# vocdoni/zk-franchise-proof-circuit

Measured on AMD Instinct MI355X. Metric: zkCensus proofs/sec (nLevels=160), higher is better.
Workload: dtype u256 (8 x u32 Montgomery, BN254 Fr/Fq)

## Files before the change

### zk-franchise-proof-circuit_amd/csrc/zkc_f29.h

```cpp
#pragma once
#include "zkc_field.h"

namespace zkc {

constexpr uint32_t F29_MASK = (1u << 29) - 1;
struct L9 { uint32_t l[9]; };

namespace f29_detail {
struct Big { uint64_t d[10]; };
constexpr Big big_norm(Big a) { uint64_t c = 0; for (int i = 0; i < 10; i++) { uint64_t v = a.d[i] + c; a.d[i] = v & F29_MASK; c = v >> 29; } return a; }
constexpr bool big_ge(const Big& a, const Big& b) { for (int i = 9; i >= 0; i--) { if (a.d[i] != b.d[i]) return a.d[i] > b.d[i]; } return true; }
constexpr Big big_sub(Big a, const Big& b) {
    int64_t br = 0;
    for (int i = 0; i < 10; i++) { int64_t v = (int64_t)a.d[i] - (int64_t)b.d[i] - br; br = v < 0; a.d[i] = (uint64_t)(v + (br ? (int64_t)1 << 29 : 0)); }
    return a;
}
constexpr Big big_shl1(Big a) { for (int i = 0; i < 10; i++) a.d[i] <<= 1; return big_norm(a); }
template <class P> constexpr Big big_p() { Big r{}; for (int k = 0; k < 9; k++) r.d[k] = P29<P>::limb(k); return r; }
template <class P> constexpr Big big_mod(Big a) {
    Big sh[40] = {}; sh[0] = big_p<P>(); int top = 0;
    for (int s = 1; s < 36; s++) { sh[s] = big_shl1(sh[s - 1]); top = s; }
    for (int s = top; s >= 0; s--) if (big_ge(a, sh[s])) a = big_sub(a, sh[s]);
    return a;
}
}

template <class P> constexpr L9 f29_p() { L9 r{}; for (int k = 0; k < 9; k++) r.l[k] = P29<P>::limb(k); return r; }
template <class P> constexpr L9 f29_dominator(uint32_t minlimb, uint32_t toplimb) {
    using namespace f29_detail;
    Big t{}; for (int i = 0; i < 8; i++) t.d[i] = minlimb; t.d[8] = toplimb;
    Big r = big_mod<P>(big_norm(t));
    bool zero = true; for (int i = 0; i < 10; i++) zero = zero && r.d[i] == 0;
    Big delta = zero ? r : big_sub(big_p<P>(), r);
    L9 o{}; for (int i = 0; i < 8; i++) o.l[i] = minlimb + (uint32_t)delta.d[i]; o.l[8] = toplimb + (uint32_t)delta.d[8];
    return o;
}
template <class P> constexpr L9 f29_pow2(int k) {
    using namespace f29_detail;
    Big t{}; t.d[k / 29] = 1ull << (k % 29);
    Big r = big_mod<P>(t);
    L9 o{}; for (int i = 0; i < 9; i++) o.l[i] = (uint32_t)r.d[i];
    return o;
}

template <class P> struct F29K {
    static constexpr L9 p = f29_p<P>();
    static constexpr L9 one = f29_pow2<P>(261);
    static constexpr L9 dom1 = f29_dominator<P>(1u << 29, 1u << 27);
    static constexpr L9 dom3 = f29_dominator<P>(3u << 29, 1u << 27);
    static constexpr uint32_t ninv = P::inv & F29_MASK;
    static constexpr uint32_t pinv = (0u - P::inv) & F29_MASK;
};

ZKC_HD void f29_from_fp_shl5(uint32_t r[9], const uint32_t a[8]) {
    r[0] = slice29<-5>(a); r[1] = slice29<24>(a); r[2] = slice29<53>(a); r[3] = slice29<82>(a); r[4] = slice29<111>(a);
    r[5] = slice29<140>(a); r[6] = slice29<169>(a); r[7] = slice29<198>(a); r[8] = slice29<227>(a);
}
ZKC_HD void f29_carry(uint32_t a[9]) {
#pragma unroll
    for (int k = 0; k < 8; k++) { a[k + 1] += a[k] >> 29; a[k] &= F29_MASK; }
}
ZKC_HD void f29_add(uint32_t r[9], const uint32_t a[9], const uint32_t b[9]) {
#pragma unroll
    for (int k = 0; k < 9; k++) r[k] = a[k] + b[k];
}
ZKC_HD void f29_sub(uint32_t r[9], const uint32_t a[9], const uint32_t b[9], const L9& D) {
#pragma unroll
    for (int k = 0; k < 9; k++) r[k] = a[k] + D.l[k] - b[k];
}

template <class P>
ZKC_HD void f29_mul(uint32_t r[9], const uint32_t a[9], const uint32_t b[9]) {
    constexpr L9 Pl = F29K<P>::p;
    uint64_t c[18];
#pragma unroll
    for (int k = 0; k < 18; k++) c[k] = 0;
#pragma unroll
    for (int i = 0; i < 9; i++)
#pragma unroll
        for (int j = 0; j < 9; j++) c[i + j] += (uint64_t)a[i] * b[j];
    uint64_t carry = 0;
#pragma unroll
    for (int i = 0; i < 9; i++) {
        c[i] += carry;
        const uint32_t m = ((uint32_t)c[i] * F29K<P>::ninv) & F29_MASK;
#pragma unroll
        for (int j = 0; j < 9; j++) c[i + j] += (uint64_t)m * Pl.l[j];
        carry = c[i] >> 29;
    }
#pragma unroll
    for (int k = 9; k < 17; k++) { c[k] += carry; r[k - 9] = (uint32_t)c[k] & F29_MASK; carry = c[k] >> 29; }
    r[8] = (uint32_t)(c[17] + carry);
}
template <class P>
ZKC_HD void f29_sqr(uint32_t r[9], const uint32_t a[9]) {
    constexpr L9 Pl = F29K<P>::p;
    uint64_t c[18];
    uint32_t a2[9];
#pragma unroll
    for (int k = 0; k < 9; k++) a2[k] = a[k] << 1;
#pragma unroll
    for (int k = 0; k < 18; k++) c[k] = 0;
#pragma unroll
    for (int i = 0; i < 9; i++) {
        c[2 * i] += (uint64_t)a[i] * a[i];
#pragma unroll
        for (int j = i + 1; j < 9; j++) c[i + j] += (uint64_t)a2[i] * a[j];
    }
    uint64_t carry = 0;
#pragma unroll
    for (int i = 0; i < 9; i++) {
        c[i] += carry;
        const uint32_t m = ((uint32_t)c[i] * F29K<P>::ninv) & F29_MASK;
#pragma unroll
        for (int j = 0; j < 9; j++) c[i + j] += (uint64_t)m * Pl.l[j];
        carry = c[i] >> 29;
    }
#pragma unroll
    for (int k = 9; k < 17; k++) { c[k] += carry; r[k - 9] = (uint32_t)c[k] & F29_MASK; carry = c[k] >> 29; }
    r[8] = (uint32_t)(c[17] + carry);
}

template <class P>
ZKC_HD void f29_reduce_cols(uint32_t r[9], uint64_t c[18]) {
    constexpr L9 Pl = F29K<P>::p;
    uint64_t carry = 0;
#pragma unroll
    for (int i = 0; i < 9; i++) {
        c[i] += carry;
        const uint32_t m = ((uint32_t)c[i] * F29K<P>::ninv) & F29_MASK;
#pragma unroll
        for (int j = 0; j < 9; j++) c[i + j] += (uint64_t)m * Pl.l[j];
        carry = c[i] >> 29;
    }
#pragma unroll
    for (int k = 9; k < 17; k++) { c[k] += carry; r[k - 9] = (uint32_t)c[k] & F29_MASK; carry = c[k] >> 29; }
    r[8] = (uint32_t)(c[17] + carry);
}
template <class P>
ZKC_HD void f29_mul_addhi(uint32_t r[9], const uint32_t a[9], const uint32_t b[9], const uint32_t h[9]) {
    uint64_t c[18];
#pragma unroll
    for (int k = 0; k < 9; k++) { c[k] = 0; c[9 + k] = h[k]; }
#pragma unroll
    for (int i = 0; i < 9; i++)
#pragma unroll
        for (int j = 0; j < 9; j++) c[i + j] += (uint64_t)a[i] * b[j];
    f29_reduce_cols<P>(r, c);
}
template <class P>
ZKC_HD void f29_sqr_addhi(uint32_t r[9], const uint32_t a[9], const uint32_t h[9]) {
    uint64_t c[18]; uint32_t a2[9];
#pragma unroll
    for (int k = 0; k < 9; k++) { a2[k] = a[k] << 1; c[k] = 0; c[9 + k] = h[k]; }
#pragma unroll
    for (int i = 0; i < 9; i++) {
        c[2 * i] += (uint64_t)a[i] * a[i];
#pragma unroll
        for (int j = i + 1; j < 9; j++) c[i + j] += (uint64_t)a2[i] * a[j];
    }
    f29_reduce_cols<P>(r, c);
}
template <class P>
ZKC_HD void f29_mul2sum_addhi(uint32_t r[9], const uint32_t a1[9], const uint32_t b1[9], const uint32_t a2[9], const uint32_t b2[9], const uint32_t h[9]) {
    uint64_t c[18];
#pragma unroll
    for (int k = 0; k < 9; k++) { c[k] = 0; c[9 + k] = h[k]; }
#pragma unroll
    for (int i = 0; i < 9; i++)
#pragma unroll
        for (int j = 0; j < 9; j++) c[i + j] += (uint64_t)a1[i] * b1[j] + (uint64_t)a2[i] * b2[j];
    f29_reduce_cols<P>(r, c);
}
template <class P>
ZKC_HD void f29_mul2sum(uint32_t r[9], const uint32_t a1[9], const uint32_t b1[9], const uint32_t a2[9], const uint32_t b2[9]) {
    uint64_t c[18];
#pragma unroll
    for (int k = 0; k < 18; k++) c[k] = 0;
#pragma unroll
    for (int i = 0; i < 9; i++)
#pragma unroll
        for (int j = 0; j < 9; j++) c[i + j] += (uint64_t)a1[i] * b1[j] + (uint64_t)a2[i] * b2[j];
    f29_reduce_cols<P>(r, c);
}

template <class P>
ZKC_HD bool f29_is_zero_mod_p(const uint32_t a[9]) {
    const uint32_t k = (a[0] * F29K<P>::pinv) & F29_MASK;
    if (k >= 64) return false;
    constexpr L9 Pl = F29K<P>::p;
    uint64_t carry = 0; uint32_t diff = 0;
#pragma unroll
    for (int i = 0; i < 9; i++) {
        const uint64_t v = (uint64_t)k * Pl.l[i] + carry;
        const uint32_t digit = i < 8 ? (uint32_t)v & F29_MASK : (uint32_t)v;
        carry = v >> 29; diff |= digit ^ a[i];
    }
    return diff == 0;
}

template <class P>
ZKC_HD void f29_reduce_small(uint32_t a[9]) {
    constexpr L9 Pl = F29K<P>::p;
    constexpr uint32_t ptop1 = (P::p[7] >> 8) + 1;
    constexpr uint32_t qmagic = (uint32_t)((1ull << 50) / ptop1);
    const uint32_t q = (uint32_t)(((uint64_t)a[8] * qmagic) >> 50);
    int64_t carry = 0;
#pragma unroll
    for (int k = 0; k < 9; k++) {
        const int64_t v = (int64_t)a[k] - (int64_t)((uint64_t)q * Pl.l[k]) + carry;
        a[k] = k < 8 ? (uint32_t)v & F29_MASK : (uint32_t)v;
        carry = v >> 29;
    }
}

template <int LO>
ZKC_HD uint32_t f29_word(const uint32_t d[9]) {
    constexpr int k = LO / 29, off = LO % 29;
    uint32_t w = d[k] >> off;
    if constexpr (k + 1 < 9) w |= d[k + 1] << (29 - off);
    if constexpr (k + 2 < 9 && 58 - off < 32) w |= d[k + 2] << (58 - off);
    return w;
}
template <class P>
ZKC_HD Fp<P> f29_to_fp(const uint32_t a[9]) {
    constexpr L9 Pl = F29K<P>::p;
    uint32_t t[9];
#pragma unroll
    for (int k = 0; k < 9; k++) t[k] = a[k];
    f29_carry(t);
    const uint32_t m = (t[0] * F29K<P>::ninv) & 31u;
    uint32_t d[9]; uint64_t carry = 0;
#pragma unroll
    for (int k = 0; k < 9; k++) { const uint64_t v = (uint64_t)m * Pl.l[k] + t[k] + carry; d[k] = k < 8 ? (uint32_t)v & F29_MASK : (uint32_t)v; carry = v >> 29; }
    Fp<P> r;
    r.v[0] = f29_word<5>(d); r.v[1] = f29_word<37>(d); r.v[2] = f29_word<69>(d); r.v[3] = f29_word<101>(d);
    r.v[4] = f29_word<133>(d); r.v[5] = f29_word<165>(d); r.v[6] = f29_word<197>(d); r.v[7] = f29_word<229>(d);
    fp_reduce_once<P>(r.v);
    return r;
}

}
```

### zk-franchise-proof-circuit_amd/csrc/zkc_ntt.hip

```cpp
#include "zkc_internal.h"
#include "zkc_prover.h"
#include "zkc_f29.h"

namespace zkc {

__device__ __forceinline__ Fr ld_fr(const Fr* p) {
    const uint4* d = reinterpret_cast<const uint4*>(p); uint4 a = d[0], b = d[1];
    Fr r; r.v[0] = a.x; r.v[1] = a.y; r.v[2] = a.z; r.v[3] = a.w; r.v[4] = b.x; r.v[5] = b.y; r.v[6] = b.z; r.v[7] = b.w; return r;
}
__device__ __forceinline__ void st_fr(Fr* p, const Fr& r) {
    uint4* d = reinterpret_cast<uint4*>(p);
    d[0] = make_uint4(r.v[0], r.v[1], r.v[2], r.v[3]); d[1] = make_uint4(r.v[4], r.v[5], r.v[6], r.v[7]);
}

constexpr uint32_t MV_UNIT = 0x80000000u, MV_NEG = 0x40000000u, MV_COL = 0x3fffffffu;
extern "C" __global__ void __launch_bounds__(256)
zkc_wtns_mont(const Fr* __restrict__ wtns_std, size_t wtns_stride, Fr* __restrict__ wm, size_t wm_stride, uint32_t nv) {
    const uint32_t i = blockIdx.x * blockDim.x + threadIdx.x;
    if (i >= nv) return;
    Fr r2;
#pragma unroll
    for (int k = 0; k < 8; k++) r2.v[k] = FrParams::r2[k];
    st_fr(wm + (size_t)blockIdx.y * wm_stride + i, ld_fr(wtns_std + (size_t)blockIdx.y * wtns_stride + i) * r2);
}
__device__ __forceinline__ Fr mv_term(const Fr* __restrict__ val, const Fr* __restrict__ w, const Fr* __restrict__ wm, uint32_t idx, uint32_t c) {
    if (wm && (c & MV_UNIT)) { const Fr x = ld_fr(wm + (c & MV_COL)); return (c & MV_NEG) ? fp_neg(x) : x; }
    return ld_fr(val + idx) * ld_fr(w + (c & MV_COL));
}
extern "C" __global__ void __launch_bounds__(256)
zkc_matvec_jds(const uint32_t* __restrict__ perm, const uint32_t* __restrict__ rowlen, const uint32_t* __restrict__ jdptr,
               const uint32_t* __restrict__ col, const Fr* __restrict__ val, const Fr* __restrict__ wtns_std, size_t wtns_stride,
               Fr* __restrict__ abc, int n, uint32_t nlong, const Fr* __restrict__ wm_all, size_t wm_stride) {
    const uint32_t t = blockIdx.x * blockDim.x + threadIdx.x, lane = threadIdx.x & 63u;
    const Fr* __restrict__ w = wtns_std + (size_t)blockIdx.y * wtns_stride;
    const Fr* __restrict__ wm = wm_all ? wm_all + (size_t)blockIdx.y * wm_stride : nullptr;
    Fr acc = Fr::zero();
    if ((t >> 6) < nlong) {
        const uint32_t r = t >> 6, len = rowlen[r];
        for (uint32_t k = lane; k < len; k += 64) { const uint32_t idx = jdptr[k] + r; acc = acc + mv_term(val, w, wm, idx, col[idx]); }
        for (int d = 32; d > 0; d >>= 1) {
            Fr o;
#pragma unroll
            for (int i = 0; i < 8; i++) o.v[i] = (uint32_t)__shfl_down((int)acc.v[i], d, 64);
            acc = acc + o;
        }
        if (lane == 0) st_fr(abc + (size_t)blockIdx.y * 3 * n + perm[r], acc);
        return;
    }
    const uint32_t r = t - nlong * 63u;
    if (r >= 2u * (uint32_t)n) return;
    const uint32_t len = rowlen[r];
    for (uint32_t k = 0; k < len; k++) { const uint32_t idx = jdptr[k] + r; acc = acc + mv_term(val, w, wm, idx, col[idx]); }
    st_fr(abc + (size_t)blockIdx.y * 3 * n + perm[r], acc);
}
extern "C" __global__ void __launch_bounds__(256)
zkc_pointwise_mul(Fr* __restrict__ abc, int n) {
    const int i = blockIdx.x * blockDim.x + threadIdx.x;
    Fr* a = abc + (size_t)blockIdx.y * 3 * n;
    if (i < n) st_fr(a + 2 * (size_t)n + i, ld_fr(a + i) * ld_fr(a + n + i));
}
struct JoinDom { static constexpr L9 D27 = f29_dominator<FrParams>(1u << 29, 1u << 27); };
extern "C" __global__ void __launch_bounds__(256)
zkc_join_abc(const Fr* __restrict__ abc, uint32_t* __restrict__ p_std, int n) {
    const int i = blockIdx.x * blockDim.x + threadIdx.x;
    if (i >= n) return;
    const Fr* a = abc + (size_t)blockIdx.y * 3 * n;
    const Fr av = ld_fr(a + i), bv = ld_fr(a + n + i), cv = ld_fr(a + 2 * (size_t)n + i);
    uint32_t A[9], B[9], C[9], T[9];
    f29_from_fp_shl5(A, av.v); f29_from_fp_shl5(B, bv.v); f29_from_fp_shl5(C, cv.v);
#pragma unroll
    for (int k = 0; k < 9; k++) C[k] = JoinDom::D27.l[k] - C[k];
    f29_mul_addhi<FrParams>(T, A, B, C);
    uint64_t col[18];
#pragma unroll
    for (int k = 0; k < 9; k++) { col[k] = T[k]; col[9 + k] = 0; }
    f29_reduce_cols<FrParams>(T, col);
    Fr r;
    r.v[0] = f29_word<0>(T); r.v[1] = f29_word<32>(T); r.v[2] = f29_word<64>(T); r.v[3] = f29_word<96>(T);
    r.v[4] = f29_word<128>(T); r.v[5] = f29_word<160>(T); r.v[6] = f29_word<192>(T); r.v[7] = f29_word<224>(T);
    fp_reduce_once<FrParams>(r.v);
    uint4* d = reinterpret_cast<uint4*>(p_std + 8 * ((size_t)blockIdx.y * n + i));
    d[0] = make_uint4(r.v[0], r.v[1], r.v[2], r.v[3]); d[1] = make_uint4(r.v[4], r.v[5], r.v[6], r.v[7]);
}

constexpr int NTT_TILE = 1024;
constexpr int TW29_WORDS = 12;
extern "C" __global__ void __launch_bounds__(256) zkc_tw29(const Fr* __restrict__ tw, uint32_t* __restrict__ out, uint32_t count) {
    const uint32_t i = blockIdx.x * blockDim.x + threadIdx.x;
    if (i >= count) return;
    const Fr x = ld_fr(tw + i);
    uint32_t t[9], r[9]; f29_from_fp_shl5(t, x.v); f29_mul<FrParams>(r, t, F29K<FrParams>::one.l);
    uint4* o = reinterpret_cast<uint4*>(out + (size_t)TW29_WORDS * i);
    o[0] = make_uint4(r[0], r[1], r[2], r[3]); o[1] = make_uint4(r[4], r[5], r[6], r[7]); o[2] = make_uint4(r[8], 0, 0, 0);
}
struct NttDom { static constexpr L9 D24 = f29_dominator<FrParams>(1u << 29, 1u << 24); static constexpr L9 D27 = f29_dominator<FrParams>(1u << 29, 1u << 27); };
__device__ __forceinline__ void ntt_ld_w(uint32_t w[9], const uint32_t* __restrict__ tw29, size_t e) {
    const uint4* wp = reinterpret_cast<const uint4*>(tw29 + (size_t)TW29_WORDS * e);
    const uint4 w0 = wp[0], w1 = wp[1], w2 = wp[2];
    w[0] = w0.x; w[1] = w0.y; w[2] = w0.z; w[3] = w0.w; w[4] = w1.x; w[5] = w1.y; w[6] = w1.z; w[7] = w1.w; w[8] = w2.x;
}
__device__ __forceinline__ void ntt_bfly(uint32_t* pu, uint32_t* pv, const uint32_t w[9], bool plain, bool carry) {
    uint32_t u[9], v[9], tt[9];
#pragma unroll
    for (int i = 0; i < 9; i++) { u[i] = pu[i]; v[i] = pv[i]; }
    if (plain) {
#pragma unroll
        for (int i = 0; i < 9; i++) { const uint32_t vi = v[i]; v[i] = u[i] + NttDom::D27.l[i] - vi; u[i] += vi; }
    } else {
        f29_mul<FrParams>(tt, v, w);
#pragma unroll
        for (int i = 0; i < 9; i++) { v[i] = u[i] + NttDom::D24.l[i] - tt[i]; u[i] += tt[i]; }
    }
    if (carry) { f29_carry(u); f29_carry(v); }
#pragma unroll
    for (int i = 0; i < 9; i++) { pu[i] = u[i]; pv[i] = v[i]; }
}
__device__ __forceinline__ void ntt_r4(uint32_t* p0, uint32_t* p1, uint32_t* p2, uint32_t* p3, const uint32_t wa[9], const uint32_t wb[9], const uint32_t wc[9], bool swap_mid) {
    uint32_t a[9], b[9], c[9], d[9], t[9];
#pragma unroll
    for (int i = 0; i < 9; i++) { a[i] = p0[i]; b[i] = p1[i]; c[i] = p2[i]; d[i] = p3[i]; }
    f29_mul<FrParams>(t, b, wa);
#pragma unroll
    for (int i = 0; i < 9; i++) { b[i] = a[i] + NttDom::D24.l[i] - t[i]; a[i] += t[i]; }
    f29_mul<FrParams>(t, d, wa);
#pragma unroll
    for (int i = 0; i < 9; i++) { d[i] = c[i] + NttDom::D24.l[i] - t[i]; c[i] += t[i]; }
    f29_mul<FrParams>(t, c, wb);
#pragma unroll
    for (int i = 0; i < 9; i++) { c[i] = a[i] + NttDom::D24.l[i] - t[i]; a[i] += t[i]; }
    f29_mul<FrParams>(t, d, wc);
#pragma unroll
    for (int i = 0; i < 9; i++) { d[i] = b[i] + NttDom::D24.l[i] - t[i]; b[i] += t[i]; }
    f29_carry(a); f29_carry(b); f29_carry(c); f29_carry(d);
    (void)swap_mid;
#pragma unroll
    for (int i = 0; i < 9; i++) { p0[i] = a[i]; p1[i] = b[i]; p2[i] = c[i]; p3[i] = d[i]; }
}
extern "C" __global__ void __launch_bounds__(256)
zkc_ntt_pass(const Fr* src_all, Fr* dst_all, const uint32_t* __restrict__ tw29, const Fr* __restrict__ scale,
             int logn, int s0, int b, int first) {
    const Fr* src = src_all + ((size_t)blockIdx.y << logn);
    Fr* dst = dst_all + ((size_t)blockIdx.y << logn);
    extern __shared__ uint32_t tile[];
    const int mid_n = 1 << b;
    const int lo_bits = s0;
    const int lo_t = (NTT_TILE >> b) < (1 << lo_bits) ? (NTT_TILE >> b) : (1 << lo_bits);
    const int tiles_per_hi = (1 << lo_bits) / lo_t;
    const int hi = blockIdx.x / tiles_per_hi, lo0 = (blockIdx.x % tiles_per_hi) * lo_t;
    const int elems = mid_n * lo_t;
    const size_t base = (size_t)hi << (s0 + b);
    for (int e = threadIdx.x; e < elems; e += blockDim.x) {
        const int mid = e / lo_t, l = e - mid * lo_t;
        size_t gi = base + ((size_t)mid << s0) + lo0 + l;
        if (first) gi = __brev((unsigned)gi) >> (32 - logn);
        const Fr x = ld_fr(src + gi);
        uint32_t t[9]; f29_from_fp_shl5(t, x.v);
#pragma unroll
        for (int k = 0; k < 9; k++) tile[9 * e + k] = t[k];
    }
    __syncthreads();
    int t = 1;
    auto single = [&](int t1, bool carry) {
        const int half = 1 << (t1 - 1);
        const int s = s0 + t1;
        for (int q = threadIdx.x; q < elems / 2; q += blockDim.x) {
            const int l = q % lo_t, pr = q / lo_t;
            const int j = pr & (half - 1), blk = pr >> (t1 - 1);
            const int m0 = (blk << t1) + j, m1 = m0 + half;
            const unsigned k = ((unsigned)j << s0) + lo0 + l;
            uint32_t w[9]; ntt_ld_w(w, tw29, (size_t)k << (logn - s));
            ntt_bfly(tile + 9 * (m0 * lo_t + l), tile + 9 * (m1 * lo_t + l), w, s == 1, carry);
        }
        __syncthreads();
    };
    if (s0 == 0) { single(1, true); t = 2; }
    for (; t + 1 <= b; t += 2) {
        const int half = 1 << (t - 1), s = s0 + t;
        for (int q = threadIdx.x; q < elems / 4; q += blockDim.x) {
            const int l = q % lo_t, u = q / lo_t;
            const int j = u & (half - 1), blk = u >> (t - 1);
            const int m = (blk << (t + 1)) + j;
            const unsigned k = ((unsigned)j << s0) + lo0 + l, kh = k + ((unsigned)half << s0);
            uint32_t wa[9], wb[9], wc[9];
            ntt_ld_w(wa, tw29, (size_t)k << (logn - s)); ntt_ld_w(wb, tw29, (size_t)k << (logn - s - 1)); ntt_ld_w(wc, tw29, (size_t)kh << (logn - s - 1));
            uint32_t* p = tile + 9 * (m * lo_t + l);
            ntt_r4(p, p + 9 * half * lo_t, p + 9 * 2 * half * lo_t, p + 9 * 3 * half * lo_t, wa, wb, wc, false);
        }
        __syncthreads();
    }
    if (t <= b) single(t, true);
    for (int e = threadIdx.x; e < elems; e += blockDim.x) {
        const int mid = e / lo_t, l = e - mid * lo_t;
        const size_t gi = base + ((size_t)mid << s0) + lo0 + l;
        uint32_t r[9];
#pragma unroll
        for (int k = 0; k < 9; k++) r[k] = tile[9 * e + k];
        if (scale) { const Fr sc = ld_fr(scale + gi); uint32_t s29[9], o[9]; f29_from_fp_shl5(s29, sc.v); f29_mul<FrParams>(o, r, s29);
#pragma unroll
            for (int k = 0; k < 9; k++) r[k] = o[k]; }
        else f29_reduce_small<FrParams>(r);
        st_fr(dst + gi, f29_to_fp<FrParams>(r));
    }
}

template <int RADIX, class Slot>
__device__ __forceinline__ void ntt_nr_stages(uint32_t* tile, Slot slot, int b, int lo_t, int q0, uint32_t prefix_of_l0, int prefix_per_l, const uint32_t* __restrict__ tw29, int logn, bool fresh) {
    const int mid_n = 1 << b;
    auto tw_of = [&](int q, uint32_t i) -> size_t { return q ? (size_t)((__brev(i) >> (32 - q)) << (logn - q - 1)) : (size_t)0; };
    int r = 0;
    if (fresh) {
        const int span = mid_n >> 1, pairs = span * lo_t;
        for (int x = threadIdx.x; x < pairs; x += blockDim.x) {
            const int l = x % lo_t, j = x / lo_t;
            uint32_t w[9] = {0, 0, 0, 0, 0, 0, 0, 0, 0};
            ntt_bfly(tile + 9 * slot(j, l), tile + 9 * slot(j + span, l), w, true, true);
        }
        __syncthreads();
        r = 1;
    }
    for (; RADIX >= 4 && r + 1 < b; r += 2) {
        const int q = q0 + r, span = mid_n >> (r + 1), hspan = span >> 1, units = (mid_n >> 2) * lo_t;
        for (int x = threadIdx.x; x < units; x += blockDim.x) {
            const int l = x % lo_t, u = x / lo_t;
            const int blk = u / hspan, j = u - blk * hspan;
            const int m = blk * 2 * span + j;
            const uint32_t i = ((prefix_of_l0 + (uint32_t)(prefix_per_l * l)) << r) | (uint32_t)blk;
            uint32_t wa[9], wb[9], wc[9];
            ntt_ld_w(wa, tw29, tw_of(q, i)); ntt_ld_w(wb, tw29, tw_of(q + 1, 2 * i)); ntt_ld_w(wc, tw29, tw_of(q + 1, 2 * i + 1));
            ntt_r4(tile + 9 * slot(m, l), tile + 9 * slot(m + span, l), tile + 9 * slot(m + hspan, l), tile + 9 * slot(m + span + hspan, l), wa, wb, wc, false);
        }
        __syncthreads();
    }
    for (; r < b; r++) {
        const int q = q0 + r, span = mid_n >> (r + 1), pairs = (mid_n >> 1) * lo_t;
        for (int x = threadIdx.x; x < pairs; x += blockDim.x) {
            const int l = x % lo_t, pr = x / lo_t;
            const int blk = pr / span, j = pr - blk * span;
            const int m0 = blk * 2 * span + j;
            const uint32_t i = ((prefix_of_l0 + (uint32_t)(prefix_per_l * l)) << r) | (uint32_t)blk;
            uint32_t w[9]; ntt_ld_w(w, tw29, tw_of(q, i));
            ntt_bfly(tile + 9 * slot(m0, l), tile + 9 * slot(m0 + span, l), w, false, RADIX >= 4 || (r & 1) == 1 || r == b - 1);
        }
        __syncthreads();
    }
}
template <int RADIX>
__device__ __forceinline__ void ntt_nr_head_body(const Fr* src_all, Fr* dst_all, const uint32_t* __restrict__ tw29, int logn, int q0, int b) {
    const Fr* src = src_all + ((size_t)blockIdx.y << logn);
    Fr* dst = dst_all + ((size_t)blockIdx.y << logn);
    extern __shared__ uint32_t tile[];
    const int mid_n = 1 << b, sh = logn - q0 - b, lo_t = NTT_TILE >> b, elems = mid_n * lo_t;
    const int bpp = (1 << sh) / lo_t;
    const uint32_t prefix = blockIdx.x / bpp;
    const size_t base = ((size_t)prefix << (logn - q0)) + (size_t)(blockIdx.x % bpp) * lo_t;
    for (int e = threadIdx.x; e < elems; e += blockDim.x) {
        const int mid = e / lo_t, l = e - mid * lo_t;
        const Fr x = ld_fr(src + (base + ((size_t)mid << sh) + l));
        uint32_t t[9]; f29_from_fp_shl5(t, x.v);
#pragma unroll
        for (int k = 0; k < 9; k++) tile[9 * e + k] = t[k];
    }
    __syncthreads();
    ntt_nr_stages<RADIX>(tile, [lo_t](int mid, int l) { return mid * lo_t + l; }, b, lo_t, q0, prefix, 0, tw29, logn, q0 == 0);
    for (int e = threadIdx.x; e < elems; e += blockDim.x) {
        const int mid = e / lo_t, l = e - mid * lo_t;
        uint32_t r[9];
#pragma unroll
        for (int k = 0; k < 9; k++) r[k] = tile[9 * e + k];
        f29_reduce_small<FrParams>(r);
        st_fr(dst + (base + ((size_t)mid << sh) + l), f29_to_fp<FrParams>(r));
    }
}
extern "C" __global__ void __launch_bounds__(256)
zkc_ntt_nr_head(const Fr* src_all, Fr* dst_all, const uint32_t* __restrict__ tw29, int logn, int q0, int b) { ntt_nr_head_body<1>(src_all, dst_all, tw29, logn, q0, b); }
extern "C" __global__ void __launch_bounds__(256)
zkc_ntt_nr_head_r4(const Fr* src_all, Fr* dst_all, const uint32_t* __restrict__ tw29, int logn, int q0, int b) { ntt_nr_head_body<4>(src_all, dst_all, tw29, logn, q0, b); }
extern "C" __global__ void __launch_bounds__(256)
zkc_ntt_mid(Fr* __restrict__ data_all, const uint32_t* __restrict__ tw_inv29, const uint32_t* __restrict__ tw_fwd29, const Fr* __restrict__ scale_br, int logn) {
    Fr* __restrict__ data = data_all + ((size_t)blockIdx.y << logn);
    extern __shared__ uint32_t tile[];
    constexpr int B = 9, MID = 1 << B, NSUB = NTT_TILE / MID;
    const size_t base = (size_t)blockIdx.x * NTT_TILE;
    for (int e = threadIdx.x; e < NTT_TILE; e += blockDim.x) {
        const Fr x = ld_fr(data + base + e);
        uint32_t t[9]; f29_from_fp_shl5(t, x.v);
#pragma unroll
        for (int k = 0; k < 9; k++) tile[9 * e + k] = t[k];
    }
    __syncthreads();
    ntt_nr_stages<4>(tile, [](int mid, int l) { return l * MID + mid; }, B, NSUB, logn - B, (uint32_t)blockIdx.x * NSUB, 1, tw_inv29, logn, false);
    for (int e = threadIdx.x; e < NTT_TILE; e += blockDim.x) {
        uint32_t r[9], s29[9], o[9];
#pragma unroll
        for (int k = 0; k < 9; k++) r[k] = tile[9 * e + k];
        const Fr sc = ld_fr(scale_br + base + e);
        f29_from_fp_shl5(s29, sc.v); f29_mul<FrParams>(o, r, s29);
#pragma unroll
        for (int k = 0; k < 9; k++) tile[9 * e + k] = o[k];
    }
    __syncthreads();
    for (int x = threadIdx.x; x < NTT_TILE / 2; x += blockDim.x) {
        const int l = x / (MID / 2), pr = x - l * (MID / 2);
        uint32_t w[9] = {0, 0, 0, 0, 0, 0, 0, 0, 0};
        ntt_bfly(tile + 9 * (l * MID + 2 * pr), tile + 9 * (l * MID + 2 * pr + 1), w, true, true);
    }
    __syncthreads();
    for (int t = 2; t + 1 <= B; t += 2) {
        const int half = 1 << (t - 1);
        for (int x = threadIdx.x; x < NTT_TILE / 4; x += blockDim.x) {
            const int l = x / (MID / 4), u = x - l * (MID / 4);
            const int j = u & (half - 1), blk = u >> (t - 1);
            const int m = (blk << (t + 1)) + j;
            uint32_t wa[9], wb[9], wc[9];
            ntt_ld_w(wa, tw_fwd29, (size_t)j << (logn - t)); ntt_ld_w(wb, tw_fwd29, (size_t)j << (logn - t - 1)); ntt_ld_w(wc, tw_fwd29, (size_t)(j + half) << (logn - t - 1));
            uint32_t* p = tile + 9 * (l * MID + m);
            ntt_r4(p, p + 9 * half, p + 9 * 2 * half, p + 9 * 3 * half, wa, wb, wc, false);
        }
        __syncthreads();
    }
    for (int e = threadIdx.x; e < NTT_TILE; e += blockDim.x) {
        uint32_t r[9];
#pragma unroll
        for (int k = 0; k < 9; k++) r[k] = tile[9 * e + k];
        f29_reduce_small<FrParams>(r);
        st_fr(data + base + e, f29_to_fp<FrParams>(r));
    }
}
extern "C" __global__ void __launch_bounds__(256)
zkc_bitrev_copy(const Fr* __restrict__ src, Fr* __restrict__ dst, int logn) {
    const uint32_t i = blockIdx.x * blockDim.x + threadIdx.x;
    if (i >> logn) return;
    st_fr(dst + i, ld_fr(src + (__brev(i) >> (32 - logn))));
}
int ntt_bitrev_table(zkc_ctx* ctx, const Fr* d_src, Fr** out, int logn) {
    ZKC_HIP_CHECK(ctx, hipMalloc((void**)out, sizeof(Fr) << logn));
    hipLaunchKernelGGL(zkc_bitrev_copy, dim3(((1u << logn) + 255) / 256), dim3(256), 0, ctx->stream, d_src, *out, logn);
    ZKC_HIP_CHECK(ctx, hipGetLastError());
    return ZKC_OK;
}
int ntt_pair_run(zkc_ctx* ctx, hipStream_t st, Fr* data, const uint32_t* tw_inv29, const uint32_t* tw_fwd29, const Fr* scale_br, int logn, int nvec) {
    if (logn < 12 || logn > 27) return zkc_fail(ctx, ZKC_ERR_BAD_ARG, "ntt_pair_run: 12 <= logn <= 27");
    const int bh = logn - 9;
    const int b1 = bh <= 9 ? bh : (bh + 1) / 2, b2 = bh - b1;
    const unsigned blocks = (1u << logn) / NTT_TILE;
    static const int radix = [] { const char* e = getenv("ZKC_NTT_RADIX"); return e ? atoi(e) : 4; }();
    auto head = radix >= 4 ? zkc_ntt_nr_head_r4 : zkc_ntt_nr_head;
    hipLaunchKernelGGL(head, dim3(blocks, nvec), dim3(256), (size_t)NTT_TILE * 36, st, (const Fr*)data, data, tw_inv29, logn, 0, b1);
    if (b2) hipLaunchKernelGGL(head, dim3(blocks, nvec), dim3(256), (size_t)NTT_TILE * 36, st, (const Fr*)data, data, tw_inv29, logn, b1, b2);
    hipLaunchKernelGGL(zkc_ntt_mid, dim3(blocks, nvec), dim3(256), (size_t)NTT_TILE * 36, st, data, tw_inv29, tw_fwd29, scale_br, logn);
    hipLaunchKernelGGL(zkc_ntt_pass, dim3(blocks, nvec), dim3(256), (size_t)NTT_TILE * 36, st, (const Fr*)data, data, tw_fwd29, (const Fr*)nullptr, logn, 9, b1, 0);
    if (b2) hipLaunchKernelGGL(zkc_ntt_pass, dim3(blocks, nvec), dim3(256), (size_t)NTT_TILE * 36, st, (const Fr*)data, data, tw_fwd29, (const Fr*)nullptr, logn, 9 + b1, b2, 0);
    hipError_t e = hipGetLastError();
    if (e != hipSuccess) return zkc_fail(ctx, ZKC_ERR_HIP, std::string("ntt_pair_run: ") + hipGetErrorString(e));
    return ZKC_OK;
}

int ntt_make_tw29(zkc_ctx* ctx, const Fr* d_tw, uint32_t count, uint32_t** out) {
    ZKC_HIP_CHECK(ctx, hipMalloc((void**)out, (size_t)count * TW29_WORDS * 4));
    hipLaunchKernelGGL(zkc_tw29, dim3((count + 255) / 256), dim3(256), 0, ctx->stream, d_tw, *out, count);
    ZKC_HIP_CHECK(ctx, hipGetLastError());
    ZKC_HIP_CHECK(ctx, hipStreamSynchronize(ctx->stream));
    return ZKC_OK;
}

int ntt_run(zkc_ctx* ctx, hipStream_t st, const Fr* src, Fr* dst, const uint32_t* tw29, const Fr* scale, int logn, int nvec) {
    int s0 = 0; bool first = true;
    while (s0 < logn) {
        int b = logn - s0 < 9 ? logn - s0 : 9;
        if (logn - s0 > 9 && logn - s0 < 18) b = (logn - s0 + 1) / 2;
        if (b > 9) b = 9;
        const int lo_t = (NTT_TILE >> b) < (1 << s0) ? (NTT_TILE >> b) : (1 << s0);
        const int nblocks = (1 << logn) / ((1 << b) * lo_t);
        const bool last = s0 + b == logn;
        hipLaunchKernelGGL(zkc_ntt_pass, dim3(nblocks, nvec), dim3(256), (size_t)(1 << b) * lo_t * 36, st,
                           first ? src : dst, dst, tw29, last ? scale : nullptr, logn, s0, b, first ? 1 : 0);
        hipError_t e = hipGetLastError();
        if (e != hipSuccess) return zkc_fail(ctx, ZKC_ERR_HIP, std::string("zkc_ntt_pass: ") + hipGetErrorString(e));
        s0 += b; first = false;
    }
    return ZKC_OK;
}

}
```

### zk-franchise-proof-circuit_amd/csrc/zkc_prove.hip

```cpp
#include "zkc_prover.h"
#include "zkc_fixedbase.h"
#include "zkc_hostparse.h"
#include <cstring>
#include <ctime>
#include <cstdio>
#include <algorithm>
#include <atomic>

using namespace zkc;

extern "C" __global__ void zkc_matvec_jds(const uint32_t*, const uint32_t*, const uint32_t*, const uint32_t*, const Fr*, const Fr*, size_t, Fr*, int, uint32_t, const Fr*, size_t);
extern "C" __global__ void zkc_wtns_mont(const Fr*, size_t, Fr*, size_t, uint32_t);
extern "C" __global__ void zkc_pointwise_mul(Fr*, int);
extern "C" __global__ void zkc_join_abc(const Fr*, uint32_t*, int);
static void matvec_launch(zkc_zkey* zk, zkc_lane& L, const uint32_t* d_wtns0, int nb, hipStream_t mv) {
    const uint32_t n = zk->n, nv = zk->nVars;
    static const bool unit_off = [] { const char* e = getenv("ZKC_MATVEC_UNITS"); return e && atoi(e) == 0; }();
    const bool units = zk->n_unit_coeffs > 0 && nv <= 3 * (size_t)n && !unit_off;
    if (units) hipLaunchKernelGGL(zkc_wtns_mont, dim3((nv + 255) / 256, nb), dim3(256), 0, mv, (const Fr*)d_wtns0, (size_t)nv, L.d_t, 3 * (size_t)n, nv);
    hipLaunchKernelGGL(zkc_matvec_jds, dim3((2 * n + 63 * zk->nlong + 255) / 256, nb), dim3(256), 0, mv, zk->d_perm, zk->d_rowlen, zk->d_jdptr, zk->d_col, zk->d_val,
                       (const Fr*)d_wtns0, (size_t)nv, L.d_abc, (int)n, zk->nlong, units ? (const Fr*)L.d_t : (const Fr*)nullptr, 3 * (size_t)n);
    hipLaunchKernelGGL(zkc_pointwise_mul, dim3((n + 255) / 256, nb), dim3(256), 0, mv, L.d_abc, (int)n);
}
static constexpr uint32_t MATVEC_LONG = 16;

namespace {
uint32_t rd32(const uint8_t* p) { uint32_t v; memcpy(&v, p, 4); return v; }
uint64_t rd64(const uint8_t* p) { uint64_t v; memcpy(&v, p, 8); return v; }
G1Affine rd_g1(const uint8_t* p) { G1Affine a; memcpy(a.x.v, p, 32); memcpy(a.y.v, p + 32, 32); return a; }
G2Affine rd_g2(const uint8_t* p) { G2Affine a; memcpy(a.x.c0.v, p, 32); memcpy(a.x.c1.v, p + 32, 32); memcpy(a.y.c0.v, p + 64, 32); memcpy(a.y.c1.v, p + 96, 32); return a; }
Fr fr_root_of_unity(int logn) {
    uint32_t e[8]; for (int i = 0; i < 8; i++) e[i] = FrParams::p[i]; e[0] -= 1;
    for (int i = 0; i < 8; i++) e[i] = (e[i] >> 28) | (i < 7 ? e[i + 1] << 4 : 0);
    Fr g = fp_from_u32<FrParams>(5), w = Fr::one();
    for (int i = 255; i >= 0; i--) { w = w * w; if ((e[i >> 5] >> (i & 31)) & 1) w = w * g; }
    for (int i = 28; i > logn; i--) w = w * w;
    return w;
}
template <class T> int dmalloc(zkc_ctx* ctx, T** p, size_t count) { ZKC_HIP_CHECK(ctx, hipMalloc((void**)p, count * sizeof(T))); return ZKC_OK; }
void g1_to_std(uint8_t* out, const G1Affine& a) { uint32_t s[8]; fp_to_std<FqParams>(s, a.x); memcpy(out, s, 32); fp_to_std<FqParams>(s, a.y); memcpy(out + 32, s, 32); }
void g2_to_std(uint8_t* out, const G2Affine& a) {
    uint32_t s[8]; fp_to_std<FqParams>(s, a.x.c0); memcpy(out, s, 32); fp_to_std<FqParams>(s, a.x.c1); memcpy(out + 32, s, 32);
    fp_to_std<FqParams>(s, a.y.c0); memcpy(out + 64, s, 32); fp_to_std<FqParams>(s, a.y.c1); memcpy(out + 96, s, 32);
}
}

uint32_t* zkc_get_template(zkc_ctx* ctx, int nLevels);
int zkc_lane_streams(zkc_ctx* ctx, int l, bool with_red, zkc_ctx::LaneStreams* out);

extern "C" __global__ void __launch_bounds__(64)
zkc_fold_check(WitnessLayout L, const uint32_t* __restrict__ wtns, const uint32_t* __restrict__ tmpl, uint32_t* __restrict__ flags, int B) {
    const int n = L.n, g = blockIdx.x, tree = blockIdx.y, b = blockIdx.z;
    const int blk = tree == 0 ? L.off_census : L.off_sikver;
    int start, end;
    if (g < n - 1) {
        const int nctrl = (g == n - 3) + (g > 0 && g < n - 2) + 1;
        start = blk + L.lvl_off(g) + nctrl; end = blk + (g + 1 < n - 1 ? L.lvl_off(g + 1) : L.lvl_off(n - 1));
    } else { start = blk + L.off_n2bold; end = start + 253 + 127 + 133; }
    const uint4* w = reinterpret_cast<const uint4*>(wtns + (size_t)b * L.nWires * 8) + 2 * (size_t)start;
    const uint4* t = reinterpret_cast<const uint4*>(tmpl) + 2 * (size_t)start;
    uint32_t diff = 0;
    for (int i = threadIdx.x; i < 2 * (end - start); i += 64) { uint4 x = w[i], y = t[i]; diff |= (x.x ^ y.x) | (x.y ^ y.y) | (x.z ^ y.z) | (x.w ^ y.w); }
    const unsigned long long any = __ballot(diff != 0);
    if (threadIdx.x == 0) flags[((size_t)b * 2 + tree) * n + g] = any ? 1u : 0u;
}

extern "C" __global__ void __launch_bounds__(64)
zkc_input_depths(const uint32_t* __restrict__ inputs, int nInputs, int n, uint32_t* __restrict__ out) {
    const int b = blockIdx.x, tree = blockIdx.y;
    const uint32_t* sib = inputs + ((size_t)b * nInputs + 12 + (size_t)tree * n) * 8;
    int d = 0;
    for (int i = threadIdx.x; i < n; i += 64) {
        const uint4* q = reinterpret_cast<const uint4*>(sib + 8 * (size_t)i); const uint4 x = q[0], y = q[1];
        if (x.x | x.y | x.z | x.w | y.x | y.y | y.z | y.w) d = i + 1;
    }
    for (int m = 32; m >= 1; m >>= 1) { const int o = __shfl_xor(d, m, 64); d = o > d ? o : d; }
    if (threadIdx.x == 0) out[2 * b + tree] = (uint32_t)d;
}

extern "C" void zkc_zkey_free(zkc_zkey* zk) {
    if (!zk) return;
    ZKC_LOCK(zk->ctx);
    (void)hipSetDevice(zk->ctx->device);
    (void)hipStreamSynchronize(zk->ctx->stream);
    void* ptrs[] = {zk->d_perm, zk->d_rowlen, zk->d_jdptr, zk->d_col, zk->d_val, zk->d_tw_fwd, zk->d_tw_inv, zk->d_tw_fwd29, zk->d_tw_inv29, zk->d_coset, zk->d_coset_br, zk->d_g1, zk->d_g2, zk->d_g2_29, zk->d_g2_29_lone, zk->d_g2_29_deep,
                    zk->d_tblDelta1, zk->d_tblAlpha1, zk->d_tblBeta1, zk->d_tblDelta2, zk->d_fb4, zk->d_fb4g2, zk->d_depths};
    for (void* p : ptrs) if (p) (void)hipFree(p);
    for (auto& kv : zk->fold.vmaps) if (kv.second.d) (void)hipFree(kv.second.d);
    for (void* q : {(void*)zk->fold.d_foldA, (void*)zk->fold.d_foldB1, (void*)zk->fold.d_foldC, (void*)zk->fold.d_foldB2}) if (q) (void)hipFree(q);
    if (zk->h_depths) (void)hipHostFree(zk->h_depths);
    for (auto& c : zk->call) { for (void* q : {(void*)c.d_rs, (void*)c.d_proofs, (void*)c.d_flags, (void*)c.d_status3}) if (q) (void)hipFree(q); if (c.h_flags) (void)hipHostFree(c.h_flags); if (c.h_out) (void)hipHostFree(c.h_out); if (c.h_rs) (void)hipHostFree(c.h_rs); if (c.h_xyzz) (void)hipHostFree(c.h_xyzz); if (c.h_early) (void)hipHostFree(c.h_early); if (c.d_xyzz) (void)hipFree(c.d_xyzz); for (hipEvent_t e : c.ev_done) if (e) (void)hipEventDestroy(e); for (hipEvent_t e : c.ev_chunk) (void)hipEventDestroy(e); }
    if (zk->ctx->lanes) for (int l = 0; l < zk->nlanes; l++) for (hipStream_t q : {zk->ctx->lanes[l].st, zk->ctx->lanes[l].st2, zk->ctx->lanes[l].fin, zk->ctx->lanes[l].red}) if (q) (void)hipStreamSynchronize(q);
    delete zk;
}

static size_t dev_free_bytes() { size_t f = 0, t = 0; if (hipMemGetInfo(&f, &t) != hipSuccess) { (void)hipGetLastError(); return 0; } return f; }
static int fold_prepare(zkc_zkey* zk);
static int fb4_prepare(zkc_zkey* zk);
struct LaneNeed { size_t abc, p, fin, bs, e1, b1, e2, b2; int j1, j2; };
static LaneNeed lane_need(const zkc_zkey* zk, int inflight) {
    const uint32_t n = zk->n, nv = zk->nVars; const int NWS = msm_nw(zk->c_sec), NWB = msm_nw(zk->c_h);
    const size_t per_proof_entries = (size_t)NWS * 3 * nv + (size_t)NWB * n;
    const size_t per_proof_buckets = 3 * (size_t)msm_half(std::max(zk->c_sec, zk->c_deep)) + msm_half(zk->c_h);
    LaneNeed nd; nd.abc = 3 * (size_t)n * inflight; nd.p = 8 * (size_t)n * inflight; nd.fin = finalize_scratch_bytes(inflight); nd.bs = 2 * 2 * 8 * (size_t)nv;
    nd.e1 = per_proof_entries * inflight; nd.b1 = per_proof_buckets * inflight; nd.j1 = 4 * inflight;
    nd.e2 = (size_t)NWS * nv * inflight; nd.b2 = (size_t)msm_half(std::max(zk->c_sec, zk->c_deep)) * inflight; nd.j2 = inflight;
    return nd;
}
static bool lane_holds(const zkc_lane& L, const LaneNeed& nd) {
    return L.cap_abc >= nd.abc && L.cap_p >= nd.p && L.cap_fin >= nd.fin && L.cap_bs >= nd.bs && L.w1.max_entries >= nd.e1 && L.w1.max_buckets >= nd.b1 && L.w1.max_jobs >= nd.j1 &&
           L.w2.max_entries >= nd.e2 && L.w2.max_buckets >= nd.b2 && L.w2.max_jobs >= nd.j2;
}
static void lane_release(zkc_lane& L) {
    for (void** q : {(void**)&L.d_abc, (void**)&L.d_t, (void**)&L.d_p, &L.d_fin, (void**)&L.d_bs}) if (*q) { (void)hipFree(*q); *q = nullptr; }
    msm_work_free(L.w1); msm_work_free(L.w2);
    L.cap_abc = L.cap_p = L.cap_fin = L.cap_bs = 0; L.bytes = 0;
}
static zkc_lane* ctx_lanes(zkc_ctx* ctx) { if (!ctx->lanes) ctx->lanes = new zkc_lane[MAX_LANES]; return ctx->lanes; }
static size_t ctx_work_bytes(const zkc_ctx* ctx) { size_t t = 0; if (ctx->lanes) for (int l = 0; l < MAX_LANES; l++) t += ctx->lanes[l].bytes; return t; }
void zkc_ctx_lanes_destroy(zkc_ctx* ctx) {
    if (!ctx->lanes) return;
    for (int l = 0; l < MAX_LANES; l++) {
        zkc_lane& L = ctx->lanes[l];
        lane_release(L);
        for (hipEvent_t e : {L.ev_msm, L.ev_msm2, L.ev_sorted, L.ev_ntt, L.ev_mv, L.ev_acc, L.ev_fin[0], L.ev_fin[1], L.ev_red}) if (e) (void)hipEventDestroy(e);
    }
    delete[] ctx->lanes; ctx->lanes = nullptr;
}
static int lane_init(zkc_ctx* ctx, int l) {
    zkc_lane& L = ctx_lanes(ctx)[l];
    if (L.made) return ZKC_OK;
    static const bool red_wanted = [] { const char* e = getenv("ZKC_REDUCE_STREAM"); return e && atoi(e) == 1; }();
    zkc_ctx::LaneStreams ls; int rc = zkc_lane_streams(ctx, l, red_wanted, &ls); if (rc) return rc;
    L.st = ls.st; L.st2 = ls.st2; L.fin = ls.fin; L.red = ls.red;
    for (hipEvent_t* e : {&L.ev_msm, &L.ev_msm2, &L.ev_sorted, &L.ev_ntt, &L.ev_mv, &L.ev_acc, &L.ev_fin[0], &L.ev_fin[1], &L.ev_red}) if (!*e) ZKC_HIP_CHECK(ctx, hipEventCreateWithFlags(e, hipEventDisableTiming));
    L.made = true; return ZKC_OK;
}
struct LaneSt { hipStream_t st, st2, fin, red; };
static LaneSt lane_st(const zkc_zkey* zk, const zkc_lane& L) { hipStream_t c = zk->ctx->stream; return zk->serial_streams ? LaneSt{c, c, c, c} : LaneSt{L.st, L.st2, L.fin, L.red}; }
static int lane_ensure(zkc_zkey* zk, int l, int inflight) {
    zkc_ctx* ctx = zk->ctx; int rc;
    if ((rc = lane_init(ctx, l))) return rc;
    zkc_lane& L = ctx->lanes[l];
    inflight = std::max(1, std::min(inflight, zk->max_inflight));
    if (lane_holds(L, lane_need(zk, inflight))) return ZKC_OK;
    inflight = std::min(inflight <= 4 ? 4 : zk->max_inflight, zk->max_inflight);
    LaneNeed nd = lane_need(zk, inflight);
    nd.abc = std::max(nd.abc, L.cap_abc); nd.p = std::max(nd.p, L.cap_p); nd.fin = std::max(nd.fin, L.cap_fin); nd.bs = std::max(nd.bs, L.cap_bs);
    nd.e1 = std::max(nd.e1, L.w1.max_entries); nd.b1 = std::max(nd.b1, L.w1.max_buckets); nd.j1 = std::max(nd.j1, L.w1.max_jobs);
    nd.e2 = std::max(nd.e2, L.w2.max_entries); nd.b2 = std::max(nd.b2, L.w2.max_buckets); nd.j2 = std::max(nd.j2, L.w2.max_jobs);
    for (hipStream_t q : {L.st, L.st2, L.fin, L.red}) if (q) ZKC_HIP_CHECK(ctx, hipStreamSynchronize(q));
    ZKC_HIP_CHECK(ctx, hipStreamSynchronize(ctx->stream));
    lane_release(L);
    const size_t free_before = dev_free_bytes();
    const char* fail_at = getenv("ZKC_TEST_FAIL_ALLOC");
    rc = (fail_at && inflight >= atoi(fail_at)) ? zkc_fail(ctx, ZKC_ERR_HIP, "lanes_ensure: allocation failure injected by ZKC_TEST_FAIL_ALLOC") : ZKC_OK;
    if (!rc) rc = dmalloc(ctx, &L.d_abc, nd.abc);
    if (!rc) rc = dmalloc(ctx, &L.d_t, nd.abc);
    if (!rc) rc = dmalloc(ctx, &L.d_p, nd.p);
    if (!rc && hipMalloc(&L.d_fin, nd.fin) != hipSuccess) rc = zkc_fail(ctx, ZKC_ERR_HIP, "lanes_ensure: hipMalloc failed (blinding scratch)");
    if (!rc) rc = dmalloc(ctx, &L.d_bs, nd.bs);
    if (!rc) rc = msm_work_alloc(ctx, L.w1, nd.e1, nd.b1, nd.j1, false);
    if (!rc) rc = msm_work_alloc(ctx, L.w2, nd.e2, nd.b2, nd.j2, true);
    if (rc) { (void)hipGetLastError(); lane_release(L); return rc; }
    L.cap_abc = nd.abc; L.cap_p = nd.p; L.cap_fin = nd.fin; L.cap_bs = nd.bs;
    { const size_t f = dev_free_bytes(); L.bytes = free_before > f ? free_before - f : 0; }
    return ZKC_OK;
}
static int lanes_ensure(zkc_zkey* zk, int inflight, int first = 0, int count = -1) {
    if (count < 0) count = zk->nlanes - first;
    for (int l = first; l < first + count && l < zk->nlanes; l++) { const int rc = lane_ensure(zk, l, inflight); if (rc) return rc; }
    return ZKC_OK;
}
extern "C" int zkc_zkey_load(zkc_ctx* ctx, const void* zkey_bytes, size_t len, zkc_zkey** out) { return zkc::zkey_load_opts(ctx, zkey_bytes, len, 0, 0, out); }
size_t zkc::zkey_device_bytes(const zkc_zkey* zk, size_t* tables, size_t* work) {
    if (!zk) return 0;
    const size_t w = ctx_work_bytes(zk->ctx);
    if (tables) *tables = zk->bytes_tables; if (work) *work = w;
    return zk->bytes_tables + w;
}
int zkc::zkey_load_opts(zkc_ctx* ctx, const void* zkey_bytes, size_t len, int opt_lanes, int opt_inflight, zkc_zkey** out) {
    if (!ctx || !zkey_bytes || !out) return zkc_fail(ctx, ZKC_ERR_BAD_ARG, "zkc_zkey_load: bad argument");
    ZKC_LOCK(ctx);
    ZKC_HIP_CHECK(ctx, hipSetDevice(ctx->device));
    const size_t free_at_entry = dev_free_bytes(), work_at_entry = ctx_work_bytes(ctx);
    const uint8_t* buf = (const uint8_t*)zkey_bytes;
    parse::BinSections bs; parse::ZkeyHeader zh; std::string perr;
    if (!parse::binfile_sections(buf, len, "zkey", 1, bs, perr) || !parse::zkey_check(bs, zh, perr)) return zkc_fail(ctx, ZKC_ERR_FORMAT, perr);
    const uint8_t* const* sec = bs.sec;
    const uint8_t* h = sec[2];
    zkc_zkey* zk = new zkc_zkey(); zk->ctx = ctx;
    zk->nVars = zh.nVars; zk->nPub = zh.nPub; zk->n = zh.n; zk->logn = zh.logn; zk->nCoeffs = zh.nCoeffs;
    parse::sha256(buf, len, zk->sha256); parse::zkey_fingerprint(buf, len, bs, zk->fingerprint);
    const uint32_t n = zk->n, nv = zk->nVars, np = zk->nPub, nc = nv - np - 1;
    zk->alpha1 = rd_g1(h + 84); zk->beta1 = rd_g1(h + 148); zk->beta2 = rd_g2(h + 212); zk->gamma2 = rd_g2(h + 340);
    zk->delta1 = rd_g1(h + 468); zk->delta2 = rd_g2(h + 532);
    for (uint32_t i = 0; i <= np; i++) zk->ic.push_back(rd_g1(sec[3] + 64ull * i));
    {
        auto zero64 = [](const uint8_t* q) { for (int i = 0; i < 64; i++) if (q[i]) return false; return true; };
        zk->fold.infA.resize(nv); zk->fold.infB.resize(nv); zk->fold.infC.assign(nv, 0);
        for (uint32_t i = 0; i < nv; i++) { zk->fold.infA[i] = zero64(sec[5] + 64ull * i); zk->fold.infB[i] = zero64(sec[6] + 64ull * i); if (i > np) zk->fold.infC[i] = zero64(sec[8] + 64ull * (i - np - 1)); }
    }
    if (np == 8 && !getenv("ZKC_NO_FOLD")) for (int nl = 3; nl <= 253; nl++) if ((uint32_t)WitnessLayout::make(nl).nWires == nv) { zk->nLevels = nl; break; }
    int rc = ZKC_OK;
    auto bail = [&](int code) { zkc_zkey_free(zk); return code; };
#define ZKC_HIP_BAIL(call)                                                                                      \
    do { hipError_t _e = (call); if (_e != hipSuccess) return bail(zkc_fail(ctx, ZKC_ERR_HIP, std::string(#call) + ": " + hipGetErrorString(_e))); } while (0)
#define ZKC_UP(dst, src, bytes) ZKC_HIP_BAIL(hipMemcpy((dst), (src), (bytes), hipMemcpyHostToDevice))
    {
        std::vector<uint32_t> rowptr(2 * (size_t)n + 1, 0), col(zk->nCoeffs); std::vector<Fr> val(zk->nCoeffs);
        const uint8_t* c = sec[4] + 4;
        for (uint32_t i = 0; i < zk->nCoeffs; i++) {
            uint32_t m = rd32(c + 44ull * i), cc = rd32(c + 44ull * i + 4), s = rd32(c + 44ull * i + 8);
            rowptr[(size_t)m * n + cc + 1]++;
        }
        for (size_t r = 0; r < 2 * (size_t)n; r++) rowptr[r + 1] += rowptr[r];
        std::vector<uint32_t> fill(rowptr.begin(), rowptr.end() - 1);
        for (uint32_t i = 0; i < zk->nCoeffs; i++) {
            uint32_t m = rd32(c + 44ull * i), cc = rd32(c + 44ull * i + 4), s = rd32(c + 44ull * i + 8);
            uint32_t k = fill[(size_t)m * n + cc]++;
            col[k] = s; memcpy(val[k].v, c + 44ull * i + 12, 32);
        }
        const size_t nrows = 2 * (size_t)n;
        std::vector<uint32_t> perm(nrows), rowlen(nrows);
        for (size_t r = 0; r < nrows; r++) perm[r] = (uint32_t)r;
        std::stable_sort(perm.begin(), perm.end(), [&](uint32_t a, uint32_t b) { return rowptr[a + 1] - rowptr[a] > rowptr[b + 1] - rowptr[b]; });
        for (size_t r = 0; r < nrows; r++) rowlen[r] = rowptr[perm[r] + 1] - rowptr[perm[r]];
        const uint32_t maxlen = nrows ? rowlen[0] : 0;
        zk->nlong = 0; while (zk->nlong < nrows && rowlen[zk->nlong] > MATVEC_LONG) zk->nlong++;
        std::vector<uint32_t> jdptr(maxlen + 1, 0);
        { size_t live = nrows; for (uint32_t k = 0; k < maxlen; k++) { while (live > 0 && rowlen[live - 1] <= k) live--; jdptr[k + 1] = jdptr[k] + (uint32_t)live; } }
        std::vector<uint32_t> jcol(zk->nCoeffs); std::vector<Fr> jval(zk->nCoeffs);
        if (nv >= (1u << 30)) return bail(zkc_fail(ctx, ZKC_ERR_FORMAT, "zkey too large for 30-bit wire indices"));
        Fr one_r2, neg_r2; for (int i = 0; i < 8; i++) one_r2.v[i] = FrParams::r2[i];
        neg_r2 = Fr::zero() - one_r2;
        zk->n_unit_coeffs = 0;
        for (size_t r = 0; r < nrows; r++) for (uint32_t k = 0; k < rowlen[r]; k++) {
            const size_t dst = (size_t)jdptr[k] + r, src = (size_t)rowptr[perm[r]] + k;
            uint32_t c = col[src];
            if (val[src] == one_r2) { c |= 0x80000000u; zk->n_unit_coeffs++; } else if (val[src] == neg_r2) { c |= 0xc0000000u; zk->n_unit_coeffs++; }
            jcol[dst] = c; jval[dst] = val[src];
        }
        if ((rc = dmalloc(ctx, &zk->d_perm, nrows)) || (rc = dmalloc(ctx, &zk->d_rowlen, nrows)) || (rc = dmalloc(ctx, &zk->d_jdptr, jdptr.size())) ||
            (rc = dmalloc(ctx, &zk->d_col, jcol.size() + 1)) || (rc = dmalloc(ctx, &zk->d_val, jval.size() + 1))) return bail(rc);
        ZKC_UP(zk->d_perm, perm.data(), nrows * 4); ZKC_UP(zk->d_rowlen, rowlen.data(), nrows * 4); ZKC_UP(zk->d_jdptr, jdptr.data(), jdptr.size() * 4);
        ZKC_UP(zk->d_col, jcol.data(), jcol.size() * 4);
        ZKC_UP(zk->d_val, jval.data(), jval.size() * sizeof(Fr));
    }
    {
        const Fr w = fr_root_of_unity((int)zk->logn), g = fr_root_of_unity((int)zk->logn + 1);
        const Fr wi = fp_inv<FrParams>(w), ninv = fp_inv<FrParams>(fp_from_u32<FrParams>(n));
        std::vector<Fr> f(n / 2), b(n / 2), cs(n);
        f[0] = b[0] = Fr::one(); for (uint32_t i = 1; i < n / 2; i++) { f[i] = f[i - 1] * w; b[i] = b[i - 1] * wi; }
        cs[0] = ninv; for (uint32_t i = 1; i < n; i++) cs[i] = cs[i - 1] * g;
        if ((rc = dmalloc(ctx, &zk->d_tw_fwd, n / 2)) || (rc = dmalloc(ctx, &zk->d_tw_inv, n / 2)) || (rc = dmalloc(ctx, &zk->d_coset, n))) return bail(rc);
        ZKC_UP(zk->d_tw_fwd, f.data(), f.size() * sizeof(Fr));
        ZKC_UP(zk->d_tw_inv, b.data(), b.size() * sizeof(Fr));
        ZKC_UP(zk->d_coset, cs.data(), cs.size() * sizeof(Fr));
        if ((rc = ntt_make_tw29(ctx, zk->d_tw_fwd, n / 2, &zk->d_tw_fwd29)) || (rc = ntt_make_tw29(ctx, zk->d_tw_inv, n / 2, &zk->d_tw_inv29))) return bail(rc);
        if ((rc = ntt_bitrev_table(ctx, zk->d_coset, &zk->d_coset_br, (int)zk->logn))) return bail(rc);
    }
    auto c_for = [](size_t W) { return msm_c_for(W); };
    { const char* e_c = getenv("ZKC_C_SECTIONS"); zk->c_sec = e_c ? std::max(8, std::min(atoi(e_c), MSM_C_BIG)) : zk->nLevels >= 0 ? MSM_C_SMALL : c_for(nv); }
    { const char* e_h = getenv("ZKC_C_H"); zk->c_h = e_h ? std::max(8, std::min(atoi(e_h), MSM_C_BIG)) : zk->nLevels >= 0 ? MSM_C_BIG : std::max(c_for(n), n >= 12000 ? 15 : 12); }
    const int NWS = msm_nw(zk->c_sec);
    { const char* e_d = getenv("ZKC_DEEP_TABLES"); const int dt = e_d ? atoi(e_d) : 1; const char* e_c = getenv("ZKC_C_DEEP");
      const int cd = e_c ? std::max(13, std::min(atoi(e_c), MSM_C_BIG)) : c_for(dt == 2 ? (size_t)40000 : (size_t)nv * 4 / 5);
      zk->c_deep = (zk->nLevels >= 0 && (nv >= (1u << 16) || dt == 2) && zk->c_sec < cd && dt != 0) ? cd : 0; }
    zk->c_h = std::max(zk->c_h, std::max(zk->c_sec, zk->c_deep));
    const int NWB = msm_nw(zk->c_h);
    zk->offA = 0; zk->offB1 = NWS * nv; zk->offC = 2 * NWS * nv; zk->offH = 2 * NWS * nv + NWS * nc;
    const int NWD = zk->c_deep ? msm_nw(zk->c_deep) : 0;
    zk->offA_deep = zk->offH + NWB * n; zk->offB1_deep = zk->offA_deep + NWD * nv; zk->offC_deep = zk->offB1_deep + NWD * nv;
    const size_t g1_points = (size_t)NWS * (2 * (size_t)nv + nc) + (size_t)NWB * n + (size_t)NWD * (2 * (size_t)nv + nc);
    if (g1_points >= (1ull << 31)) return bail(zkc_fail(ctx, ZKC_ERR_FORMAT, "zkey too large for 31-bit point indices"));
    if ((rc = dmalloc(ctx, &zk->d_g1, g1_points)) || (rc = dmalloc(ctx, &zk->d_g2, (size_t)NWS * nv))) return bail(rc);
    ZKC_UP(zk->d_g1 + zk->offA, sec[5], 64ull * nv); ZKC_UP(zk->d_g1 + zk->offB1, sec[6], 64ull * nv);
    ZKC_UP(zk->d_g1 + zk->offC, sec[8], 64ull * nc); ZKC_UP(zk->d_g1 + zk->offH, sec[9], 64ull * n);
    ZKC_UP(zk->d_g2, sec[7], 128ull * nv);
    if ((rc = msm_precompute_g1(ctx, nv, zk->d_g1 + zk->offA, zk->c_sec)) || (rc = msm_precompute_g1(ctx, nv, zk->d_g1 + zk->offB1, zk->c_sec)) ||
        (rc = msm_precompute_g1(ctx, nc, zk->d_g1 + zk->offC, zk->c_sec)) || (rc = msm_precompute_g1(ctx, n, zk->d_g1 + zk->offH, zk->c_h)) ||
        (rc = msm_precompute_g2(ctx, nv, zk->d_g2, zk->c_sec))) return bail(rc);
    if ((rc = dmalloc(ctx, &zk->d_g2_29, 60 * (size_t)NWS * nv)) || (rc = msm_g2_table29(ctx, zk->d_g2, zk->d_g2_29, (size_t)NWS * nv))) return bail(rc);
    if (zk->c_deep) {
        ZKC_UP(zk->d_g1 + zk->offA_deep, sec[5], 64ull * nv); ZKC_UP(zk->d_g1 + zk->offB1_deep, sec[6], 64ull * nv); ZKC_UP(zk->d_g1 + zk->offC_deep, sec[8], 64ull * nc);
        if ((rc = msm_precompute_g1(ctx, nv, zk->d_g1 + zk->offA_deep, zk->c_deep)) || (rc = msm_precompute_g1(ctx, nv, zk->d_g1 + zk->offB1_deep, zk->c_deep)) ||
            (rc = msm_precompute_g1(ctx, nc, zk->d_g1 + zk->offC_deep, zk->c_deep))) return bail(rc);
        G2Affine* tmp = nullptr;
        if ((rc = dmalloc(ctx, &tmp, (size_t)NWD * nv))) return bail(rc);
        hipError_t e2 = hipMemcpyAsync(tmp, zk->d_g2, 128ull * nv, hipMemcpyDeviceToDevice, ctx->stream);
        if (e2 == hipSuccess) rc = msm_precompute_g2(ctx, nv, tmp, zk->c_deep);
        if (e2 == hipSuccess && !rc) rc = dmalloc(ctx, &zk->d_g2_29_deep, 60 * (size_t)NWD * nv);
        if (e2 == hipSuccess && !rc) rc = msm_g2_table29(ctx, tmp, zk->d_g2_29_deep, (size_t)NWD * nv);
        if (e2 == hipSuccess && !rc) e2 = hipStreamSynchronize(ctx->stream);
        (void)hipFree(tmp);
        if (rc) return bail(rc);
        if (e2 != hipSuccess) return bail(zkc_fail(ctx, ZKC_ERR_HIP, std::string("second section tables: ") + hipGetErrorString(e2)));
    }
    {
        const char* e_lone = getenv("ZKC_G2_LONE_TABLE");
        if (!(e_lone && atoi(e_lone) == 0) && (zk->nLevels >= 0 || nv < (1u << 16))) {
            constexpr int NWL = msm_nw(MSM_C_G2_LONE);
            G2Affine* tmp = nullptr;
            if ((rc = dmalloc(ctx, &tmp, (size_t)NWL * nv))) return bail(rc);
            hipError_t e2 = hipMemcpyAsync(tmp, zk->d_g2, 128ull * nv, hipMemcpyDeviceToDevice, ctx->stream);
            if (e2 == hipSuccess) rc = msm_precompute_g2(ctx, nv, tmp, MSM_C_G2_LONE);
            if (e2 == hipSuccess && !rc) rc = dmalloc(ctx, &zk->d_g2_29_lone, 60 * (size_t)NWL * nv);
            if (e2 == hipSuccess && !rc) rc = msm_g2_table29(ctx, tmp, zk->d_g2_29_lone, (size_t)NWL * nv);
            if (e2 == hipSuccess && !rc) e2 = hipStreamSynchronize(ctx->stream);
            (void)hipFree(tmp);
            if (rc) return bail(rc);
            if (e2 != hipSuccess) return bail(zkc_fail(ctx, ZKC_ERR_HIP, std::string("lone-proof G2 table: ") + hipGetErrorString(e2)));
        }
    }
    const char* e_inf = getenv("ZKC_INFLIGHT");
    zk->max_inflight = opt_inflight > 0 ? std::min(opt_inflight, MSM_MAX_JOBS / 4) : e_inf ? std::max(1, std::min(atoi(e_inf), MSM_MAX_JOBS / 4)) : zk->nLevels >= 0 ? 64 : 96;
    {
        const size_t per_proof_entries = (size_t)NWS * 3 * nv + (size_t)NWB * n, census_pass = 96ull * (22ull * 3 * 82754 + 15ull * 131072);
        const int fit = (int)std::max<size_t>(1, census_pass / std::max<size_t>(per_proof_entries, 1));
        zk->max_inflight = std::min(zk->max_inflight, fit);
    }
    { const char* e_l = getenv("ZKC_LANES"); zk->nlanes = opt_lanes > 0 ? std::min(opt_lanes, (int)MAX_LANES) : e_l ? std::max(1, std::min(atoi(e_l), (int)MAX_LANES)) : zk->nLevels >= 0 ? (int)MAX_LANES : 1; }
    zk->serial_streams = getenv("ZKC_SERIAL_STREAMS") != nullptr;
    if ((rc = lanes_ensure(zk, 1, 0, 1))) return bail(rc);
    {
        FixedBase<Fq> td(zk->delta1), ta(zk->alpha1), tb(zk->beta1); FixedBase<Fq2> t2(zk->delta2);
        if ((rc = dmalloc(ctx, &zk->d_tblDelta1, td.tab.size())) || (rc = dmalloc(ctx, &zk->d_tblAlpha1, ta.tab.size())) ||
            (rc = dmalloc(ctx, &zk->d_tblBeta1, tb.tab.size())) || (rc = dmalloc(ctx, &zk->d_tblDelta2, t2.tab.size()))) return bail(rc);
        ZKC_UP(zk->d_tblDelta1, td.tab.data(), td.tab.size() * sizeof(G1Affine)); ZKC_UP(zk->d_tblAlpha1, ta.tab.data(), ta.tab.size() * sizeof(G1Affine));
        ZKC_UP(zk->d_tblBeta1, tb.tab.data(), tb.tab.size() * sizeof(G1Affine)); ZKC_UP(zk->d_tblDelta2, t2.tab.data(), t2.tab.size() * sizeof(G2Affine));
    }
    ZKC_HIP_BAIL(hipStreamSynchronize(ctx->stream));
    if (zk->nLevels >= 0 && (rc = fold_prepare(zk))) return bail(rc);
    if ((rc = fb4_prepare(zk))) return bail(rc);
    { const size_t f = dev_free_bytes(), grown = ctx_work_bytes(ctx) > work_at_entry ? ctx_work_bytes(ctx) - work_at_entry : 0; zk->bytes_tables = free_at_entry > f + grown ? free_at_entry - f - grown : 0; }
    *out = zk;
    return ZKC_OK;
#undef ZKC_UP
#undef ZKC_HIP_BAIL
}

int zkc::prove_reserve(zkc_zkey* zk, int inflight) {
    if (!zk) return ZKC_ERR_BAD_ARG;
    ZKC_LOCK(zk->ctx);
    ZKC_HIP_CHECK(zk->ctx, hipSetDevice(zk->ctx->device));
    return lanes_ensure(zk, inflight);
}
extern "C" int zkc_zkey_pass_info(const zkc_zkey* zk, int* pass_size, int* lanes) {
    if (!zk) return ZKC_ERR_BAD_ARG;
    if (pass_size) *pass_size = zk->max_inflight; if (lanes) *lanes = zk->nlanes;
    return ZKC_OK;
}
extern "C" int zkc_zkey_info(const zkc_zkey* zk, uint32_t* nVars, uint32_t* nPublic, uint32_t* domainSize) {
    if (!zk) return ZKC_ERR_BAD_ARG;
    if (nVars) *nVars = zk->nVars; if (nPublic) *nPublic = zk->nPub; if (domainSize) *domainSize = zk->n;
    return ZKC_OK;
}

static std::vector<std::pair<int, int>> fold_group_ranges(const WitnessLayout& L, int tree) {
    std::vector<std::pair<int, int>> r; const int n = L.n, blk = tree == 0 ? L.off_census : L.off_sikver;
    for (int g = 0; g < n - 1; g++) {
        const int nctrl = (g == n - 3) + (g > 0 && g < n - 2) + 1;
        r.push_back({blk + L.lvl_off(g) + nctrl, blk + (g + 1 < n - 1 ? L.lvl_off(g + 1) : L.lvl_off(n - 1))});
    }
    r.push_back({blk + L.off_n2bold, blk + L.off_n2bold + 253 + 127 + 133});
    return r;
}
template <class X> static void suffix_sums(std::vector<X>& suf, const X* g, int n) {
    suf.assign(n, X::inf());
    for (int D = n - 2; D >= 0; D--) suf[D] = xyzz_add(suf[D + 1], g[D]);
}
template <class PT> static int fold_upload(zkc_ctx* ctx, PT** d, const std::vector<PT>& b, const std::vector<PT>* suf) {
    std::vector<PT> t; t.push_back(b[0]); t.insert(t.end(), suf[0].begin(), suf[0].end()); t.insert(t.end(), suf[1].begin(), suf[1].end());
    ZKC_HIP_CHECK(ctx, hipMalloc((void**)d, t.size() * sizeof(PT)));
    ZKC_HIP_CHECK(ctx, hipMemcpy(*d, t.data(), t.size() * sizeof(PT), hipMemcpyHostToDevice));
    return ZKC_OK;
}
static int fold_prepare(zkc_zkey* zk) {
    if (zk->fold.ready) return ZKC_OK;
    zkc_ctx* ctx = zk->ctx; const WitnessLayout L = WitnessLayout::make(zk->nLevels); const int n = L.n;
    uint32_t* tmpl = zkc_get_template(ctx, zk->nLevels); if (!tmpl) return ZKC_ERR_HIP;
    std::vector<uint32_t> wires, gstart;
    for (int tree = 0; tree < 2; tree++) for (auto& rg : fold_group_ranges(L, tree)) { gstart.push_back((uint32_t)wires.size()); for (int w = rg.first; w < rg.second; w++) wires.push_back((uint32_t)w); }
    gstart.push_back((uint32_t)wires.size());
    const uint32_t ng = 2 * n;
    uint32_t *d_w = nullptr, *d_g = nullptr;
    ZKC_HIP_CHECK(ctx, hipMalloc((void**)&d_w, wires.size() * 4)); ZKC_HIP_CHECK(ctx, hipMalloc((void**)&d_g, gstart.size() * 4));
    ZKC_HIP_CHECK(ctx, hipMemcpy(d_w, wires.data(), wires.size() * 4, hipMemcpyHostToDevice));
    ZKC_HIP_CHECK(ctx, hipMemcpy(d_g, gstart.data(), gstart.size() * 4, hipMemcpyHostToDevice));
    std::vector<G1XYZZ> gA(ng), gB1(ng), gC(ng); std::vector<G2XYZZ> gB2(ng);
    int rc;
    if ((rc = fold_group_sums_g1(ctx, zk->d_g1 + zk->offA, tmpl, d_w, (uint32_t)wires.size(), 0, d_g, ng, gA.data())) ||
        (rc = fold_group_sums_g1(ctx, zk->d_g1 + zk->offB1, tmpl, d_w, (uint32_t)wires.size(), 0, d_g, ng, gB1.data())) ||
        (rc = fold_group_sums_g1(ctx, zk->d_g1 + zk->offC, tmpl, d_w, (uint32_t)wires.size(), (int32_t)zk->nPub + 1, d_g, ng, gC.data())) ||
        (rc = fold_group_sums_g2(ctx, zk->d_g2, tmpl, d_w, (uint32_t)wires.size(), 0, d_g, ng, gB2.data()))) return rc;
    ZKC_HIP_CHECK(ctx, hipFree(d_w)); ZKC_HIP_CHECK(ctx, hipFree(d_g));
    auto& f = zk->fold;
    for (int t = 0; t < 2; t++) {
        suffix_sums(f.sufA[t], gA.data() + t * n, n); suffix_sums(f.sufB1[t], gB1.data() + t * n, n);
        suffix_sums(f.sufC[t], gC.data() + t * n, n); suffix_sums(f.sufB2[t], gB2.data() + t * n, n);
    }
    f.baseA = {xyzz_add(gA[n - 1], gA[2 * n - 1])}; f.baseB1 = {xyzz_add(gB1[n - 1], gB1[2 * n - 1])};
    f.baseC = {xyzz_add(gC[n - 1], gC[2 * n - 1])}; f.baseB2 = {xyzz_add(gB2[n - 1], gB2[2 * n - 1])};
    if ((rc = fold_upload(ctx, &f.d_foldA, f.baseA, f.sufA)) || (rc = fold_upload(ctx, &f.d_foldB1, f.baseB1, f.sufB1)) || (rc = fold_upload(ctx, &f.d_foldC, f.baseC, f.sufC)) ||
        (rc = fold_upload(ctx, &f.d_foldB2, f.baseB2, f.sufB2))) return rc;
    f.ready = true;
    return ZKC_OK;
}
static int fb4_prepare(zkc_zkey* zk) {
    const char* e_off = getenv("ZKC_BLIND_TREE");
    if ((e_off && atoi(e_off) == 0) || zk->d_fb4) return ZKC_OK;
    zkc_ctx* ctx = zk->ctx;
    std::vector<G1XYZZ> bases = {G1XYZZ::from_affine(zk->delta1), G1XYZZ::from_affine(zk->alpha1), G1XYZZ::from_affine(zk->beta1)};
    const auto& f = zk->fold;
    if (f.ready) {
        bases.push_back(xyzz_add_affine(f.baseA[0], zk->alpha1)); bases.push_back(xyzz_add_affine(f.baseB1[0], zk->beta1));
        for (int t = 0; t < 2; t++) bases.insert(bases.end(), f.sufA[t].begin(), f.sufA[t].end());
        for (int t = 0; t < 2; t++) bases.insert(bases.end(), f.sufB1[t].begin(), f.sufB1[t].end());
    }
    G1XYZZ* d_bases = nullptr; int rc;
    if ((rc = dmalloc(ctx, &d_bases, bases.size()))) return rc;
    if ((rc = dmalloc(ctx, &zk->d_fb4, bases.size() * FB4_WIN * FB4_ROW)) || (rc = dmalloc(ctx, &zk->d_fb4g2, (size_t)FB4_WIN * FB4_ROW + 2))) { (void)hipFree(d_bases); return rc; }
    hipError_t e = hipMemcpyAsync(d_bases, bases.data(), bases.size() * sizeof(G1XYZZ), hipMemcpyHostToDevice, ctx->stream);
    if (e == hipSuccess) { rc = fb4_build(ctx, ctx->stream, d_bases, (int)bases.size(), zk->d_fb4, G2XYZZ::from_affine(zk->delta2), G2XYZZ::from_affine(zk->beta2),
                                             f.ready ? xyzz_add_affine(f.baseB2[0], zk->beta2) : G2XYZZ::from_affine(zk->beta2), zk->d_fb4g2); if (!rc) e = hipStreamSynchronize(ctx->stream); }
    (void)hipFree(d_bases);
    if (rc || e != hipSuccess) {
        (void)hipFree(zk->d_fb4); (void)hipFree(zk->d_fb4g2); zk->d_fb4 = nullptr; zk->d_fb4g2 = nullptr;
        return rc ? rc : zkc_fail(ctx, ZKC_ERR_HIP, std::string("fb4_prepare: ") + hipGetErrorString(e));
    }
    zk->fb4_bases = (int)bases.size();
    return ZKC_OK;
}
static int fold_vmap(zkc_zkey* zk, int Dc, int Ds, zkc_zkey::Fold::VMap* out) {
    auto it = zk->fold.vmaps.find({Dc, Ds});
    if (it != zk->fold.vmaps.end()) { *out = it->second; return ZKC_OK; }
    zkc_ctx* ctx = zk->ctx; const WitnessLayout L = WitnessLayout::make(zk->nLevels); const int n = L.n;
    std::vector<uint8_t> folded(L.nWires, 0);
    for (int tree = 0; tree < 2; tree++) {
        auto rg = fold_group_ranges(L, tree); const int D = tree == 0 ? Dc : Ds;
        for (int g = D; g < n - 1; g++) for (int w = rg[g].first; w < rg[g].second; w++) folded[w] = 1;
        for (int w = rg[n - 1].first; w < rg[n - 1].second; w++) folded[w] = 1;
    }
    std::vector<uint32_t> v; zkc_zkey::Fold::VMap m;
    m.offA = 0; for (int w = 0; w < L.nWires; w++) if (!folded[w] && !zk->fold.infA[w]) v.push_back((uint32_t)w); m.nA = (uint32_t)v.size();
    m.offB = (uint32_t)v.size(); for (int w = 0; w < L.nWires; w++) if (!folded[w] && !zk->fold.infB[w]) v.push_back((uint32_t)w); m.nB = (uint32_t)v.size() - m.offB;
    m.offC = (uint32_t)v.size(); for (int w = (int)zk->nPub + 1; w < L.nWires; w++) if (!folded[w] && !zk->fold.infC[w]) v.push_back((uint32_t)w); m.nC = (uint32_t)v.size() - m.offC;
    ZKC_HIP_CHECK(ctx, hipMalloc((void**)&m.d, v.size() * 4 + 4));
    ZKC_HIP_CHECK(ctx, hipMemcpyAsync(m.d, v.data(), v.size() * 4, hipMemcpyHostToDevice, ctx->stream));
    ZKC_HIP_CHECK(ctx, hipStreamSynchronize(ctx->stream));
    zk->fold.vmaps[{Dc, Ds}] = m; *out = m;
    return ZKC_OK;
}

static int nofold_vmap(zkc_zkey* zk, zkc_zkey::Fold::VMap* out) {
    auto it = zk->fold.vmaps.find({-1, -1});
    if (it != zk->fold.vmaps.end()) { *out = it->second; return ZKC_OK; }
    zkc_ctx* ctx = zk->ctx; const uint32_t nv = zk->nVars, np = zk->nPub;
    std::vector<uint32_t> v; zkc_zkey::Fold::VMap m;
    m.offA = 0; for (uint32_t w = 0; w < nv; w++) if (!zk->fold.infA[w]) v.push_back(w); m.nA = (uint32_t)v.size();
    m.offB = (uint32_t)v.size(); for (uint32_t w = 0; w < nv; w++) if (!zk->fold.infB[w]) v.push_back(w); m.nB = (uint32_t)v.size() - m.offB;
    m.offC = (uint32_t)v.size(); for (uint32_t w = np + 1; w < nv; w++) if (!zk->fold.infC[w]) v.push_back(w); m.nC = (uint32_t)v.size() - m.offC;
    if ((size_t)m.nA + m.nB + m.nC + (size_t)nv / 50 < 3 * (size_t)nv - np - 1) {
        ZKC_HIP_CHECK(ctx, hipMalloc((void**)&m.d, v.size() * 4 + 4));
        ZKC_HIP_CHECK(ctx, hipMemcpyAsync(m.d, v.data(), v.size() * 4, hipMemcpyHostToDevice, ctx->stream));
        ZKC_HIP_CHECK(ctx, hipStreamSynchronize(ctx->stream));
    }
    zk->fold.vmaps[{-1, -1}] = m; *out = m;
    return ZKC_OK;
}

static int h_matvec_dev(zkc_zkey* zk, zkc_lane& L, const uint32_t* d_wtns0, int nb, hipStream_t mv) {
    zkc_ctx* ctx = zk->ctx; const uint32_t n = zk->n, nv = zk->nVars;
    zkc_prof_scope _ps(ctx, ZKC_PROF_MATVEC, (uint64_t)nb * ((uint64_t)zk->nCoeffs * 68 + 3ull * n * 32), mv);
    matvec_launch(zk, L, d_wtns0, nb, mv);
    ZKC_HIP_CHECK(ctx, hipGetLastError());
    return ZKC_OK;
}
static int h_evals_dev(zkc_zkey* zk, zkc_lane& L, hipStream_t st, const uint32_t* d_wtns0, int nb, bool with_matvec = true) {
    zkc_ctx* ctx = zk->ctx; const uint32_t n = zk->n;
    if (with_matvec) { int rc0 = h_matvec_dev(zk, L, d_wtns0, nb, st); if (rc0) return rc0; }
    zkc_prof_scope _pn(ctx, ZKC_PROF_NTT, (uint64_t)nb * (6ull * 2 * n * 32 + 4ull * n * 32), st);
    int rc;
    static const bool ntt_two_transforms = getenv("ZKC_NTT_SEPARATE") != nullptr;
    if (!ntt_two_transforms && zk->logn >= 12 && zk->logn <= 27) {
        if ((rc = ntt_pair_run(ctx, st, L.d_abc, zk->d_tw_inv29, zk->d_tw_fwd29, zk->d_coset_br, (int)zk->logn, 3 * nb))) return rc;
    } else {
        if ((rc = ntt_run(ctx, st, L.d_abc, L.d_t, zk->d_tw_inv29, zk->d_coset, (int)zk->logn, 3 * nb))) return rc;
        if ((rc = ntt_run(ctx, st, L.d_t, L.d_abc, zk->d_tw_fwd29, nullptr, (int)zk->logn, 3 * nb))) return rc;
    }
    hipLaunchKernelGGL(zkc_join_abc, dim3((n + 255) / 256, nb), dim3(256), 0, st, L.d_abc, L.d_p, (int)n);
    ZKC_HIP_CHECK(ctx, hipGetLastError());
    return ZKC_OK;
}

extern "C" int zkc_debug_stage(zkc_zkey* zk, const void* d_wtns, int stage, void* host_out) {
    if (!zk || !d_wtns || !host_out) return ZKC_ERR_BAD_ARG;
    zkc_ctx* ctx = zk->ctx; const uint32_t n = zk->n;
    ZKC_LOCK(ctx);
    ZKC_HIP_CHECK(ctx, hipSetDevice(ctx->device)); ZKC_HIP_CHECK(ctx, hipStreamSynchronize(ctx->stream));
    { int rc0 = lanes_ensure(zk, 1, 0, 1); if (rc0) return rc0; }
    zkc_lane& L0 = ctx->lanes[0]; const hipStream_t st0 = lane_st(zk, L0).st;
    if (stage == 0) {
        matvec_launch(zk, L0, (const uint32_t*)d_wtns, 1, st0);
        ZKC_HIP_CHECK(ctx, hipGetLastError());
        ZKC_HIP_CHECK(ctx, hipMemcpyAsync(host_out, L0.d_abc, 96ull * n, hipMemcpyDeviceToHost, st0));
    } else {
        int rc = h_evals_dev(zk, L0, st0, (const uint32_t*)d_wtns, 1); if (rc) return rc;
        ZKC_HIP_CHECK(ctx, hipMemcpyAsync(host_out, L0.d_p, 32ull * n, hipMemcpyDeviceToHost, st0));
    }
    ZKC_HIP_CHECK(ctx, hipStreamSynchronize(st0));
    return ZKC_OK;
}

extern "C" int zkc_msm_debug(zkc_zkey* zk, int which, const void* d_scalars, uint32_t count, void* host_out) {
    if (!zk || !d_scalars || !host_out || which < 0 || which > 4) return ZKC_ERR_BAD_ARG;
    zkc_ctx* ctx = zk->ctx;
    ZKC_LOCK(ctx);
    ZKC_HIP_CHECK(ctx, hipSetDevice(ctx->device)); ZKC_HIP_CHECK(ctx, hipStreamSynchronize(ctx->stream));
    { int rc0 = lanes_ensure(zk, 1, 0, 1); if (rc0) return rc0; }
    zkc_lane& L0 = ctx->lanes[0]; const hipStream_t st_l0 = lane_st(zk, L0).st;
    const uint32_t full = which == 3 ? zk->nVars - zk->nPub - 1 : which == 4 ? zk->n : zk->nVars;
    if (count != full) return zkc_fail(ctx, ZKC_ERR_BAD_ARG, "zkc_msm_debug: count must equal the section size");
    static thread_local MsmJobList jl; jl.clear(256, 1024, which == 2 ? (uint32_t)MSM_MAX_VW_PER_JOB : (uint32_t)MSM_MAX_VW_G1);
    const uint32_t offs[5] = {zk->offA, zk->offB1, 0, zk->offC, zk->offH};
    jl.add((const uint32_t*)d_scalars, nullptr, count, offs[which], full, 0, which == 4 ? zk->c_h : zk->c_sec);
    int rc = which == 2 ? msm_pass_g2(zk, L0.w2, jl, 0, true, st_l0) : msm_pass_g1(zk, L0.w1, jl, 0, true, st_l0); if (rc) return rc;
    ZKC_HIP_CHECK(ctx, hipStreamSynchronize(st_l0));
    if (which == 2) g2_to_std((uint8_t*)host_out, xyzz_to_affine(*(G2XYZZ*)L0.w2.h_results));
    else g1_to_std((uint8_t*)host_out, xyzz_to_affine(*(G1XYZZ*)L0.w1.h_results));
    return ZKC_OK;
}

int zkc_witness_chunk_async(zkc_ctx* ctx, int nLevels, const void* d_inputs, int B, void* d_wtns, int32_t* d_status3, int32_t* d_status, hipStream_t st);
int zkc::prove_batch_begin(zkc_zkey* zk, int cs, const void* d_wtns, uint32_t nWitness, int B, const uint8_t* rs, bool want_publics, const void* d_inputs, int32_t* d_status,
                           int lane0, hipEvent_t wait_first, const uint8_t* host_depths, bool no_early) {
    if (!zk || !d_wtns || !rs || B <= 0 || cs < 0 || cs >= CALL_SLOTS || lane0 >= zk->nlanes) return zkc_fail(zk ? zk->ctx : nullptr, ZKC_ERR_BAD_ARG, "zkc_prove_batch_dev: bad argument");
    zkc_ctx* ctx = zk->ctx;
    ZKC_LOCK(ctx);
    if (nWitness != zk->nVars) return zkc_fail(ctx, ZKC_ERR_INVALID_WITNESS_LENGTH, "Invalid witness length. Circuit: " + std::to_string(zk->nVars) + ", witness: " + std::to_string(nWitness));
    for (int b = 0; b < 2 * B; b++) { uint32_t t[8]; memcpy(t, rs + 32 * (size_t)b, 32); if (!fp_std_lt_p<FrParams>(t)) return zkc_fail(ctx, ZKC_ERR_BAD_ARG, "r or s >= field order"); }
    ZKC_HIP_CHECK(ctx, hipSetDevice(ctx->device));
    const uint32_t nv = zk->nVars, np = zk->nPub, nc = nv - np - 1, n = zk->n;
    const bool can_fold = zk->nLevels >= 0;
    WitnessLayout L{}; int rc;
    {
        const int npasses0 = (B + zk->max_inflight - 1) / zk->max_inflight, per0 = (B + npasses0 - 1) / npasses0;
        if ((rc = lanes_ensure(zk, per0, lane0 >= 0 ? lane0 : 0, lane0 >= 0 ? 1 : std::min(zk->nlanes, npasses0)))) return rc;
    }
    hipStream_t st0 = (lane0 >= 0 && !zk->serial_streams && B <= zk->max_inflight) ? ctx->lanes[lane0].st : ctx->stream;
    zkc_zkey::CallSlot& CS = zk->call[cs];
    if (CS.pending) return zkc_fail(ctx, ZKC_ERR_BAD_ARG, "prove_batch_begin: this call slot has a call in flight (finish it first)");
    if (CS.cap < (size_t)B) {
        if (CS.d_rs) { ZKC_HIP_CHECK(ctx, hipFree(CS.d_rs)); ZKC_HIP_CHECK(ctx, hipFree(CS.d_proofs)); ZKC_HIP_CHECK(ctx, hipHostFree(CS.h_out)); ZKC_HIP_CHECK(ctx, hipHostFree(CS.h_rs)); ZKC_HIP_CHECK(ctx, hipFree(CS.d_xyzz)); ZKC_HIP_CHECK(ctx, hipHostFree(CS.h_xyzz));
                       CS.d_rs = CS.d_proofs = CS.h_out = CS.h_rs = CS.d_xyzz = CS.h_xyzz = nullptr; CS.cap = 0; }
        const size_t want = std::max<size_t>((size_t)B, std::max<size_t>(256, std::min<size_t>(2 * CS.cap, 4096)));
        ZKC_HIP_CHECK(ctx, hipMalloc((void**)&CS.d_rs, 64 * want)); ZKC_HIP_CHECK(ctx, hipMalloc((void**)&CS.d_proofs, 256 * want));
        ZKC_HIP_CHECK(ctx, hipHostMalloc((void**)&CS.h_out, (256 + 32 * (size_t)zk->nPub) * want)); ZKC_HIP_CHECK(ctx, hipHostMalloc((void**)&CS.h_rs, 64 * want));
        ZKC_HIP_CHECK(ctx, hipMalloc((void**)&CS.d_xyzz, 512 * want)); ZKC_HIP_CHECK(ctx, hipHostMalloc((void**)&CS.h_xyzz, 512 * want)); CS.cap = want;
    }
    static const unsigned ev_host_flags = hipEventDisableTiming;
    for (int l = 0; l < zk->nlanes; l++) if (!CS.ev_done[l]) ZKC_HIP_CHECK(ctx, hipEventCreateWithFlags(&CS.ev_done[l], ev_host_flags));
    CS.as_xyzz.assign((size_t)B, 0); CS.lanes_used = 0;
    if (wait_first) ZKC_HIP_CHECK(ctx, hipStreamWaitEvent(st0, wait_first, 0));
    uint8_t* const h_pub = CS.h_out + 256ull * CS.cap;
    if (rs != CS.h_rs_copy.data()) CS.h_rs_copy.assign(rs, rs + 64 * (size_t)B);
    memcpy(CS.h_rs, rs, 64 * (size_t)B);
    ZKC_HIP_CHECK(ctx, hipMemcpyAsync(CS.d_rs, CS.h_rs, 64 * (size_t)B, hipMemcpyHostToDevice, st0));
    uint32_t* tmpl = nullptr;
    if (can_fold) {
        L = WitnessLayout::make(zk->nLevels);
        if ((rc = fold_prepare(zk))) return rc;
        tmpl = zkc_get_template(ctx, zk->nLevels); if (!tmpl) return ZKC_ERR_HIP;
        const size_t nflags = (size_t)B * 2 * L.n;
        if (CS.flags_cap < nflags) {
            if (CS.d_flags) { ZKC_HIP_CHECK(ctx, hipFree(CS.d_flags)); ZKC_HIP_CHECK(ctx, hipHostFree(CS.h_flags)); CS.d_flags = CS.h_flags = nullptr; CS.flags_cap = 0; }
            const size_t want = std::max(nflags, (size_t)256 * 2 * L.n);
            ZKC_HIP_CHECK(ctx, hipMalloc((void**)&CS.d_flags, want * 4)); ZKC_HIP_CHECK(ctx, hipHostMalloc((void**)&CS.h_flags, want * 4)); CS.flags_cap = want;
        }
    }
    CS.early_n = 0; CS.arg_wtns = d_wtns; CS.arg_nw = nWitness; CS.arg_publics = want_publics; CS.arg_lane0 = lane0; CS.arg_inputs = d_inputs != nullptr; CS.arg_wait = nullptr;
    static const bool early_any = [] { const char* e = getenv("ZKC_EARLY_LAYOUT"); return !(e && atoi(e) == 0); }();
    const size_t ecap = MSM_MAX_JOBS / 4;
    const bool early_wanted = !no_early && can_fold && B <= zk->max_inflight && (B <= 2 ? zk->d_fb4 != nullptr : early_any);
    if (early_wanted && !CS.h_early) { ZKC_HIP_CHECK(ctx, hipHostMalloc((void**)&CS.h_early, (ecap + ecap * 2 * 256) * 4)); CS.early_cap = ecap; }
    if (early_wanted && host_depths) {
        bool ok = true; for (int i = 0; i < 2 * B; i++) ok = ok && host_depths[i] < (uint8_t)L.n && L.n <= 255;
        if (ok) { CS.early_n = B; CS.early_depth.assign(host_depths, host_depths + 2 * (size_t)B); }
    } else if (early_wanted && d_inputs) {
        if (!zk->d_depths) { ZKC_HIP_CHECK(ctx, hipMalloc((void**)&zk->d_depths, 2 * ecap * 4)); ZKC_HIP_CHECK(ctx, hipHostMalloc((void**)&zk->h_depths, 2 * ecap * 4)); }
        uint32_t* hd = zk->h_depths;
        if (wait_first) ZKC_HIP_CHECK(ctx, hipStreamWaitEvent(ctx->stream2, wait_first, 0));
        hipLaunchKernelGGL(zkc_input_depths, dim3(B, 2), dim3(64), 0, ctx->stream2, (const uint32_t*)d_inputs, L.nInputs, L.n, zk->d_depths);
        ZKC_HIP_CHECK(ctx, hipGetLastError());
        ZKC_HIP_CHECK(ctx, hipMemcpyAsync(hd, zk->d_depths, 8 * (size_t)B, hipMemcpyDeviceToHost, ctx->stream2));
        ZKC_HIP_CHECK(ctx, hipStreamSynchronize(ctx->stream2));
        bool ok = true; for (int i = 0; i < 2 * B; i++) ok = ok && hd[i] < (uint32_t)L.n;
        if (ok) { CS.early_n = B; CS.early_depth.resize(2 * (size_t)B); for (int i = 0; i < 2 * B; i++) CS.early_depth[i] = (uint8_t)hd[i]; }
    }
    const int npasses = (B + zk->max_inflight - 1) / zk->max_inflight;
    const int per_pass = (B + npasses - 1) / npasses;
    while ((int)CS.ev_chunk.size() < npasses) { hipEvent_t e; ZKC_HIP_CHECK(ctx, hipEventCreateWithFlags(&e, ev_host_flags)); CS.ev_chunk.push_back(e); }
    int32_t* d_status3 = nullptr;
    if (d_inputs) {
        if ((rc = zkc_ensure(ctx, (void**)&CS.d_status3, &CS.status3_cap, std::max<size_t>((size_t)B, 256) * 3 * sizeof(int32_t)))) return rc;
        d_status3 = CS.d_status3;
    }
    static const int wgroup = [] { const char* e = getenv("ZKC_WITNESS_GROUP"); return e ? std::max(1, atoi(e)) : 8; }();
    for (int c = 0; c < npasses; c++) {
        const int p0 = c * per_pass, nb = std::min(per_pass, B - p0);
        uint32_t* wc = (uint32_t*)d_wtns + (size_t)p0 * nv * 8;
        if (d_inputs && (c % wgroup == 0 || c == 1)) {
            const int glast = c == 0 ? 1 : std::min(((c / wgroup) + 1) * wgroup, npasses);
            const int g0 = p0, gn = std::min((glast - c) * per_pass, B - g0);
            if (gn > 0 && (rc = zkc_witness_chunk_async(ctx, zk->nLevels, (const uint8_t*)d_inputs + (size_t)g0 * L.nInputs * 32, gn, wc, d_status3 + 3 * (size_t)g0, d_status + g0, st0))) return rc;
        }
        if (can_fold) {
            uint32_t* fl = CS.d_flags + (size_t)p0 * 2 * L.n;
            hipLaunchKernelGGL(zkc_fold_check, dim3(L.n, 2, nb), dim3(64), 0, st0, L, (const uint32_t*)wc, tmpl, fl, nb);
            ZKC_HIP_CHECK(ctx, hipGetLastError());
            ZKC_HIP_CHECK(ctx, hipMemcpyAsync(CS.h_flags + (size_t)p0 * 2 * L.n, fl, (size_t)nb * 2 * L.n * 4, hipMemcpyDeviceToHost, st0));
        }
        if (CS.early_n) {
            if (d_status) ZKC_HIP_CHECK(ctx, hipMemcpyAsync(CS.h_early, d_status, 4 * (size_t)B, hipMemcpyDeviceToHost, st0));
            else memset(CS.h_early, 0, 4 * (size_t)B);
            ZKC_HIP_CHECK(ctx, hipMemcpyAsync(CS.h_early + CS.early_cap, CS.d_flags + (size_t)p0 * 2 * L.n, (size_t)nb * 2 * L.n * 4, hipMemcpyDeviceToHost, st0));
        }
        ZKC_HIP_CHECK(ctx, hipEventRecord(CS.ev_chunk[c], st0));
    }
    static const bool trace_host = getenv("ZKC_TRACE_HOST") != nullptr;
    auto now_ms = [] { timespec t; clock_gettime(CLOCK_MONOTONIC, &t); return t.tv_sec * 1e3 + t.tv_nsec * 1e-6; };
    const double t_begin = now_ms(); double tr[6] = {0};
    int pass = 0, done_on_st_lane = -1;
    const bool one_lane = lane0 >= 0 || zk->nlanes == 1;
    for (int p0 = 0; p0 < B; p0 += per_pass, pass++) {
        const int nb = std::min(per_pass, B - p0);
        const int li = lane0 >= 0 ? lane0 : pass % zk->nlanes; CS.lanes_used |= 1u << li;
        zkc_lane& LN = ctx->lanes[li]; const LaneSt LS = lane_st(zk, LN); const int slot = LN.npass & 1;
        tr[0] = now_ms();
        const bool early = CS.early_n > 0;
        if (!early) ZKC_HIP_CHECK(ctx, zkc_wait_event(CS.ev_chunk[pass]));
        tr[1] = now_ms();
        ZKC_HIP_CHECK(ctx, hipStreamWaitEvent(LS.st, CS.ev_chunk[pass], 0)); ZKC_HIP_CHECK(ctx, hipStreamWaitEvent(LS.st2, CS.ev_chunk[pass], 0));
        hipStream_t st = LS.st, st2 = LS.st2, fin = LS.fin;
        const uint32_t* w0 = (const uint32_t*)d_wtns + (size_t)p0 * nv * 8;
        uint8_t dcq[MSM_MAX_JOBS / 4], dsq[MSM_MAX_JOBS / 4]; bool fold = can_fold;
        if (early) for (int q = 0; q < nb; q++) { dcq[q] = CS.early_depth[2 * q]; dsq[q] = CS.early_depth[2 * q + 1]; }
        else for (int q = 0; q < nb && fold; q++) for (int t = 0; t < 2; t++) {
            const uint32_t* f = CS.h_flags + ((size_t)(p0 + q) * 2 + t) * L.n;
            if (f[L.n - 1]) { fold = false; break; }
            int D = 0; for (int g = 0; g < L.n - 1; g++) if (f[g]) D = g + 1;
            (t == 0 ? dcq : dsq)[q] = (uint8_t)D;
        }
        static thread_local zkc_zkey::Fold::VMap vms[MSM_MAX_JOBS / 4];
        if (fold) for (int q = 0; q < nb; q++) if ((rc = fold_vmap(zk, dcq[q], dsq[q], &vms[q]))) return rc;
        static const bool nofold_lists = [] { const char* e = getenv("ZKC_NOFOLD_LISTS"); return !(e && atoi(e) == 0); }();
        if (!fold && nofold_lists) {
            zkc_zkey::Fold::VMap nf; if ((rc = nofold_vmap(zk, &nf))) return rc;
            for (int q = 0; q < nb; q++) vms[q] = nf;
        }
        const bool listed = fold || (nofold_lists && vms[0].d != nullptr);
        if (LN.npass >= 2) { ZKC_HIP_CHECK(ctx, hipStreamWaitEvent(st, LN.ev_fin[slot], 0)); ZKC_HIP_CHECK(ctx, hipStreamWaitEvent(st2, LN.ev_fin[slot], 0)); }
        LN.npass++;
        static const bool mv_prefetch_env = getenv("ZKC_MATVEC_INLINE") == nullptr;
        const bool mv_prefetch = mv_prefetch_env && one_lane;
        const bool mv_done = mv_prefetch && pass > 0;
        if (mv_done) ZKC_HIP_CHECK(ctx, hipStreamWaitEvent(st, LN.ev_mv, 0));
        if ((rc = h_evals_dev(zk, LN, st, w0, nb, !mv_done))) return rc;
        ZKC_HIP_CHECK(ctx, hipEventRecord(LN.ev_ntt, st));
        tr[2] = now_ms();
        static thread_local MsmJobList j1, j2;
        static const uint32_t vwb_env = [] { const char* e = getenv("ZKC_VW_BIG"); return e ? (uint32_t)atoi(e) : 0u; }();
        static const uint32_t vws_env = [] { const char* e = getenv("ZKC_VW_SMALL"); return e ? (uint32_t)atoi(e) : 0u; }();
        const uint32_t vws = nb <= 4 ? 64u : vws_env ? vws_env : nb < 32 ? 256u : 2048u, vwb = nb <= 4 ? 256u : vwb_env ? vwb_env : nb < 32 ? 1024u : 4096u;
        size_t lone_entries = 0; for (int q = 0; q < nb; q++) lone_entries += (size_t)msm_nw(MSM_C_G2_LONE) * (listed ? vms[q].nB : nv);
        static const size_t deep_wires = [] { const char* e = getenv("ZKC_DEEP_WIRES"); return e ? (size_t)atol(e) : (size_t)16000; }();
        size_t live_wires = 0; for (int q = 0; q < nb; q++) live_wires += listed ? (size_t)vms[q].nA + vms[q].nB + vms[q].nC : 2 * (size_t)nv + nc;
        const bool deep = zk->c_deep != 0 && nb > 2 && live_wires >= 3 * deep_wires * (size_t)nb;
        const int cw = deep ? zk->c_deep : zk->c_sec;
        const uint32_t oA = deep ? zk->offA_deep : zk->offA, oB1 = deep ? zk->offB1_deep : zk->offB1, oC = deep ? zk->offC_deep : zk->offC;
        const int c2 = (nb <= 2 && zk->d_g2_29_lone && lone_entries <= LN.w2.max_entries) ? MSM_C_G2_LONE : cw;
        static const uint32_t vwg2_env = [] { const char* e = getenv("ZKC_VW_G2"); return e ? (uint32_t)atoi(e) : 0u; }();
        j1.clear(vws, vwb, MSM_MAX_VW_G1); j2.clear(c2 == MSM_C_G2_LONE ? 128u : (vwg2_env && nb >= 32) ? vwg2_env : vws, 1024, MSM_MAX_VW_PER_JOB);
        for (int q = 0; q < nb; q++) j1.add(LN.d_p + 8 * (size_t)n * q, nullptr, n, zk->offH, n, 0, zk->c_h);
        size_t tree_entries = 0; for (int q = 0; q < nb; q++) tree_entries += (size_t)msm_nw(zk->c_h) * n + (size_t)msm_nw(zk->c_sec) * (listed ? 2 * (size_t)vms[q].nA + 2 * (size_t)vms[q].nB + vms[q].nC : 4 * (size_t)nv + nc);
        const bool tree = zk->d_fb4 != nullptr && nb <= 2 && 6 * nb <= LN.w1.max_jobs && tree_entries <= LN.w1.max_entries && (size_t)nb * (5 * msm_half(zk->c_sec) + msm_half(zk->c_h)) <= LN.w1.max_buckets;
        BlindArgs ba{}; ba.rs = CS.d_rs + 64 * (size_t)p0; ba.nv = nv;
        for (int q = 0; q < nb; q++) {
            const uint32_t* w = w0 + (size_t)q * nv * 8;
            uint32_t* bs = tree ? LN.d_bs + (size_t)q * 2 * nv * 8 : nullptr;
            if (tree) { ba.w[q] = w; ba.out[q] = bs; }
            if (listed) {
                const zkc_zkey::Fold::VMap& vm = vms[q];
                j1.add(w, vm.d + vm.offA, vm.nA, oA, nv, 0, cw);
                j1.add(w, vm.d + vm.offB, vm.nB, oB1, nv, 0, cw);
                j1.add(w, vm.d + vm.offC, vm.nC, oC, nc, (int32_t)np + 1, cw);
                if (tree) { j1.add(bs, vm.d + vm.offA, vm.nA, oA, nv, 0, cw); j1.add(bs + 8ull * nv, vm.d + vm.offB, vm.nB, oB1, nv, 0, cw); }
                j2.add(w, vm.d + vm.offB, vm.nB, 0, nv, 0, c2);
                if (tree) { ba.mapA[q] = vm.d + vm.offA; ba.nA[q] = vm.nA; ba.mapB[q] = vm.d + vm.offB; ba.nB[q] = vm.nB; }
            } else {
                j1.add(w, nullptr, nv, oA, nv, 0, cw);
                j1.add(w, nullptr, nv, oB1, nv, 0, cw);
                j1.add(w + 8ull * (np + 1), nullptr, nc, oC, nc, 0, cw);
                if (tree) { j1.add(bs, nullptr, nv, oA, nv, 0, cw); j1.add(bs + 8ull * nv, nullptr, nv, oB1, nv, 0, cw); }
                j2.add(w, nullptr, nv, 0, nv, 0, c2);
                if (tree) { ba.mapA[q] = ba.mapB[q] = nullptr; ba.nA[q] = ba.nB[q] = nv; }
            }
        }
        if (tree && (rc = blind_scalars_launch(ctx, st, ba, nb))) return rc;
        FinalizeArgs fa{};
        fa.r1 = (const G1XYZZ*)LN.w1.results + (size_t)slot * LN.w1.max_jobs; fa.r2 = (const G2XYZZ*)LN.w2.results + (size_t)slot * LN.w2.max_jobs;
        fa.foldA = zk->fold.d_foldA; fa.foldB1 = zk->fold.d_foldB1; fa.foldC = zk->fold.d_foldC; fa.foldB2 = zk->fold.d_foldB2; fa.fold_n = can_fold ? L.n : 0;
        for (int q = 0; q < nb; q++) { fa.dc[q] = fold ? dcq[q] : (uint8_t)255; fa.ds[q] = fold ? dsq[q] : (uint8_t)255; }
        fa.tblDelta1 = zk->d_tblDelta1; fa.tblAlpha1 = zk->d_tblAlpha1; fa.tblBeta1 = zk->d_tblBeta1; fa.tblDelta2 = zk->d_tblDelta2;
        fa.alpha1 = zk->alpha1; fa.beta2 = zk->beta2; fa.rs = CS.d_rs + 64 * (size_t)p0; fa.out = CS.d_proofs + 256 * (size_t)p0; fa.scratch = LN.d_fin;
        fa.per = tree ? 5 : 3; fa.fb4 = zk->d_fb4; fa.fb4g2 = zk->d_fb4g2; fa.out_xyzz = CS.d_xyzz + 512 * (size_t)p0;
        static const bool g2_early = getenv("ZKC_G2_LATE") == nullptr;
        static const bool g2_hold_env = getenv("ZKC_G2_ACC_HOLD") != nullptr, g2_early_env = getenv("ZKC_G2_ACC_EARLY") != nullptr;
        const bool g2_acc_with_sort = g2_hold_env || ((nb < 32 || !one_lane) && !g2_early_env);
        if (g2_early) {
            if ((rc = msm_pass_g2(zk, LN.w2, j2, slot, false, st2, g2_acc_with_sort ? LN.ev_ntt : nullptr))) return rc;
            if (tree && (rc = finalize_tree_g2_launch(ctx, st2, fa, nb))) return rc;
            ZKC_HIP_CHECK(ctx, hipEventRecord(LN.ev_msm2, st2));
        }
        tr[3] = now_ms();
        ZKC_HIP_CHECK(ctx, hipStreamWaitEvent(st, LN.ev_red, 0));
        static const bool red_on = [] { const char* e = getenv("ZKC_REDUCE_STREAM"); return e && atoi(e) == 1; }();
        const bool red_split = red_on && !zk->serial_streams && nb >= 32;
        if ((rc = msm_pass_g1(zk, LN.w1, j1, slot, false, st, LN.ev_sorted, LN.ev_acc, (red_split && LS.red) ? LS.red : nullptr, LN.ev_red))) return rc;
        tr[4] = now_ms();
        if (!g2_early) {
            ZKC_HIP_CHECK(ctx, hipStreamWaitEvent(st2, LN.ev_sorted, 0));
            if ((rc = msm_pass_g2(zk, LN.w2, j2, slot, false, st2))) return rc;
            if (tree && (rc = finalize_tree_g2_launch(ctx, st2, fa, nb))) return rc;
            ZKC_HIP_CHECK(ctx, hipEventRecord(LN.ev_msm2, st2));
        }
        if (want_publics)
            ZKC_HIP_CHECK(ctx, hipMemcpy2DAsync(h_pub + 32ull * np * p0, 32ull * np, w0 + 8, 32ull * nv, 32ull * np, nb, hipMemcpyDeviceToHost, st));
        ZKC_HIP_CHECK(ctx, hipEventRecord(LN.ev_msm, st));
        if (mv_prefetch && p0 + per_pass < B) {
            const int p1 = p0 + per_pass, nb1 = std::min(per_pass, B - p1);
            static const bool mv_at_ntt = [] { const char* e = getenv("ZKC_MV_PREFETCH_AT_NTT"); return e && atoi(e) == 1; }();
            ZKC_HIP_CHECK(ctx, hipStreamWaitEvent(fin, mv_at_ntt ? LN.ev_ntt : LN.ev_sorted, 0));
            ZKC_HIP_CHECK(ctx, hipStreamWaitEvent(fin, CS.ev_chunk[pass + 1], 0));
            if ((rc = h_matvec_dev(zk, LN, (const uint32_t*)d_wtns + (size_t)p1 * nv * 8, nb1, fin))) return rc;
            ZKC_HIP_CHECK(ctx, hipEventRecord(LN.ev_mv, fin));
        }
        hipStream_t bl = ((tree || lane0 >= 0) && npasses == 1) ? st : fin;
        if (bl == fin) { ZKC_HIP_CHECK(ctx, hipStreamWaitEvent(fin, LN.ev_msm, 0)); ZKC_HIP_CHECK(ctx, hipStreamWaitEvent(fin, LN.ev_red, 0)); }
        else { if (LN.npass >= 2) ZKC_HIP_CHECK(ctx, hipStreamWaitEvent(st, LN.ev_fin[slot ^ 1], 0)); if (red_split) ZKC_HIP_CHECK(ctx, hipStreamWaitEvent(st, LN.ev_red, 0)); }
        if (!tree) ZKC_HIP_CHECK(ctx, hipStreamWaitEvent(bl, LN.ev_msm2, 0));
        if ((rc = finalize_launch(ctx, bl, fa, nb))) return rc;
        if (tree) ZKC_HIP_CHECK(ctx, hipStreamWaitEvent(bl, LN.ev_msm2, 0));
        if (tree) { ZKC_HIP_CHECK(ctx, hipMemcpyAsync(CS.h_xyzz + 512ull * p0, CS.d_xyzz + 512 * (size_t)p0, 512ull * nb, hipMemcpyDeviceToHost, bl)); for (int q = 0; q < nb; q++) CS.as_xyzz[p0 + q] = 1; }
        else ZKC_HIP_CHECK(ctx, hipMemcpyAsync(CS.h_out + 256ull * p0, CS.d_proofs + 256 * (size_t)p0, 256ull * nb, hipMemcpyDeviceToHost, bl));
        ZKC_HIP_CHECK(ctx, hipEventRecord(LN.ev_fin[slot], bl));
        if (bl == st) done_on_st_lane = li;
        tr[5] = now_ms();
        if (trace_host) fprintf(stderr, "[zkc host] pass %2d: start %8.2f | chunk wait %6.2f | h_evals %6.2f | g2 pass %6.2f | g1 pass %6.2f | blinding %6.2f ms\n", pass, tr[0] - t_begin,
                                tr[1] - tr[0], tr[2] - tr[1], tr[3] - tr[2], tr[4] - tr[3], tr[5] - tr[4]);
    }
    for (int l = 0; l < zk->nlanes; l++) if (CS.lanes_used >> l & 1) { const LaneSt ls = lane_st(zk, ctx->lanes[l]); ZKC_HIP_CHECK(ctx, hipEventRecord(CS.ev_done[l], done_on_st_lane == l ? ls.st : ls.fin)); }
    CS.B = B; CS.pending = true;
    return ZKC_OK;
}
static std::atomic<unsigned long long> g_early_retries{0};
extern "C" unsigned long long zkc_debug_early_retries(void) { return g_early_retries.load(); }
int zkc::prove_batch_finish(zkc_zkey* zk, int cs, uint8_t* proofs, uint8_t* publics) {
    if (!zk || !proofs || cs < 0 || cs >= CALL_SLOTS) return zkc_fail(zk ? zk->ctx : nullptr, ZKC_ERR_BAD_ARG, "prove_batch_finish: bad argument");
    zkc_zkey::CallSlot& CS = zk->call[cs];
    if (!CS.pending) return zkc_fail(zk->ctx, ZKC_ERR_BAD_ARG, "prove_batch_finish: no call in flight on this slot");
    hipError_t e = hipSuccess;
    for (int l = 0; l < zk->nlanes && e == hipSuccess; l++) if (CS.lanes_used >> l & 1) e = zkc_wait_event(CS.ev_done[l], CS.B <= 2 ? 6000u : 0u);
    CS.pending = false;
    if (e != hipSuccess) { ZKC_LOCK(zk->ctx); return zkc_fail(zk->ctx, ZKC_ERR_HIP, std::string("prove_batch_finish: ") + hipGetErrorString(e)); }
    if (CS.early_n) {
        const WitnessLayout L = WitnessLayout::make(zk->nLevels);
        for (int q = 0; q < CS.early_n; q++) {
            if ((int32_t)CS.h_early[q] != ZKC_W_OK) continue;
            for (int t = 0; t < 2; t++) {
                const uint32_t* f = CS.h_early + CS.early_cap + ((size_t)q * 2 + t) * L.n;
                int D = 0; for (int g = 0; g < L.n - 1; g++) if (f[g]) D = g + 1;
                if (f[L.n - 1] || D > (int)CS.early_depth[2 * q + t]) {
                    if (!CS.arg_inputs) { g_early_retries++; int rc = prove_batch_begin(zk, cs, CS.arg_wtns, CS.arg_nw, CS.B, CS.h_rs_copy.data(), CS.arg_publics, nullptr, nullptr, CS.arg_lane0, nullptr, nullptr, true); if (rc) return rc; return prove_batch_finish(zk, cs, proofs, publics); }
                    ZKC_LOCK(zk->ctx); return zkc_fail(zk->ctx, ZKC_ERR_GENERIC, "prove_batch_finish: the witness does not fold at the depth its inputs gave (internal error)");
                }
            }
        }
    }
    memcpy(proofs, CS.h_out, 256ull * CS.B);
    for (int q = 0; q < CS.B; q++) if (CS.as_xyzz[q]) {
        const uint8_t* x = CS.h_xyzz + 512 * (size_t)q; uint8_t* o = proofs + 256 * (size_t)q;
        G1XYZZ a, c; G2XYZZ b; memcpy(&a, x, 128); memcpy(&b, x + 128, 256); memcpy(&c, x + 384, 128);
        g1_to_std(o, xyzz_to_affine_gcd(a)); g2_to_std(o + 64, xyzz_to_affine_gcd(b)); g1_to_std(o + 192, xyzz_to_affine_gcd(c));
    }
    if (publics) memcpy(publics, CS.h_out + 256ull * CS.cap, 32ull * zk->nPub * CS.B);
    return ZKC_OK;
}
static int prove_batch_impl(zkc_zkey* zk, const void* d_wtns, uint32_t nWitness, int B, const uint8_t* rs, uint8_t* proofs, uint8_t* publics,
                            const void* d_inputs, int32_t* d_status) {
    if (!zk || !proofs) return zkc_fail(zk ? zk->ctx : nullptr, ZKC_ERR_BAD_ARG, "zkc_prove_batch_dev: bad argument");
    ZKC_LOCK(zk->ctx);
    for (int c = 1; c < CALL_SLOTS; c++) if (zk->call[c].pending) return zkc_fail(zk->ctx, ZKC_ERR_BAD_ARG, "zkc_prove_batch_dev: the key has a split call in flight (proving service)");
    int rc = prove_batch_begin(zk, 0, d_wtns, nWitness, B, rs, publics != nullptr, d_inputs, d_status);
    if (rc) return rc;
    return prove_batch_finish(zk, 0, proofs, publics);
}

extern "C" int zkc_batch_begin(zkc_zkey* zk, int slot, const void* d_inputs, int B, void* d_wtns, int32_t* d_status, const uint8_t* rs) {
    if (!zk || !d_wtns || (d_inputs && !d_status) || slot < 0 || slot >= CALL_SLOTS) return zkc_fail(zk ? zk->ctx : nullptr, ZKC_ERR_BAD_ARG, "zkc_batch_begin: bad argument");
    if (d_inputs && zk->nLevels < 0) return zkc_fail(zk->ctx, ZKC_ERR_BAD_ARG, "zkc_batch_begin: the key is not a ZkFranchiseProofCircuit(nLevels) key; compute the witness elsewhere and pass d_inputs = NULL");
    return prove_batch_begin(zk, slot, d_wtns, zk->nVars, B, rs, true, d_inputs, d_status);
}
extern "C" int zkc_batch_finish(zkc_zkey* zk, int slot, uint8_t* proofs, uint8_t* publics) { return prove_batch_finish(zk, slot, proofs, publics); }

extern "C" int zkc_prove_batch_dev(zkc_zkey* zk, const void* d_wtns, uint32_t nWitness, int B, const uint8_t* rs, uint8_t* proofs, uint8_t* publics) {
    return prove_batch_impl(zk, d_wtns, nWitness, B, rs, proofs, publics, nullptr, nullptr);
}
extern "C" int zkc_fullprove_batch_dev(zkc_zkey* zk, const void* d_inputs, int B, void* d_wtns, int32_t* d_status, const uint8_t* rs, uint8_t* proofs, uint8_t* publics) {
    if (!zk || !d_inputs || !d_status) return zkc_fail(zk ? zk->ctx : nullptr, ZKC_ERR_BAD_ARG, "zkc_fullprove_batch_dev: bad argument");
    if (zk->nLevels < 0) return zkc_fail(zk->ctx, ZKC_ERR_BAD_ARG, "zkc_fullprove_batch_dev: the key is not a ZkFranchiseProofCircuit(nLevels) key; compute the witness elsewhere and call zkc_prove_batch_dev");
    return prove_batch_impl(zk, d_wtns, zk->nVars, B, rs, proofs, publics, d_inputs, d_status);
}

extern "C" int zkc_prove_dev(zkc_zkey* zk, const void* d_wtns, uint32_t nWitness, const uint8_t r32[32], const uint8_t s32[32],
                             uint8_t proof[256], uint8_t* public_out) {
    if (!r32 || !s32) return zkc_fail(zk ? zk->ctx : nullptr, ZKC_ERR_BAD_ARG, "zkc_prove_dev: bad argument");
    uint8_t rs[64]; memcpy(rs, r32, 32); memcpy(rs + 32, s32, 32);
    return zkc_prove_batch_dev(zk, d_wtns, nWitness, 1, rs, proof, public_out);
}

extern "C" int zkc_prove(zkc_zkey* zk, const void* wtns, uint32_t nWitness, const uint8_t r32[32], const uint8_t s32[32],
                         uint8_t proof[256], uint8_t* public_out) {
    if (!zk || !wtns) return zkc_fail(zk ? zk->ctx : nullptr, ZKC_ERR_BAD_ARG, "zkc_prove: bad argument");
    zkc_ctx* ctx = zk->ctx;
    ZKC_LOCK(ctx);
    if (nWitness != zk->nVars) return zkc_fail(ctx, ZKC_ERR_INVALID_WITNESS_LENGTH, "Invalid witness length. Circuit: " + std::to_string(zk->nVars) + ", witness: " + std::to_string(nWitness));
    ZKC_HIP_CHECK(ctx, hipSetDevice(ctx->device));
    int rc = zkc_ensure(ctx, &ctx->d_scratch_out, &ctx->scratch_out_sz, 32ull * nWitness); if (rc) return rc;
    ZKC_HIP_CHECK(ctx, hipMemcpyAsync(ctx->d_scratch_out, wtns, 32ull * nWitness, hipMemcpyHostToDevice, ctx->stream));
    return zkc_prove_dev(zk, ctx->d_scratch_out, nWitness, r32, s32, proof, public_out);
}
```

### zk-franchise-proof-circuit_amd/csrc/zkc_prover.h

```cpp
#pragma once
#include "zkc_internal.h"
#include "zkc_curve.h"

namespace zkc {
constexpr int MSM_C_BIG = 17, MSM_C_SMALL = 12;
constexpr int MSM_C_G2_LONE = 8;
inline int msm_c_for(size_t W) { return W < 12000 ? 12 : W < 22000 ? 13 : W < 90000 ? 15 : W < 180000 ? 16 : 17; }
constexpr int msm_nw(int c) { return (254 + c) / c; }
constexpr int msm_half(int c) { return 1 << (c - 1); }
constexpr int MSM_VW_MIN = 64, MSM_MAX_VW_PER_JOB = 64;
constexpr int MSM_MAX_VW_G1 = 256;
constexpr int MSM_SEG_MIN = 16;
#ifndef ZKC_MSM_SEG
#define ZKC_MSM_SEG 128
#endif
constexpr int MSM_SEG = ZKC_MSM_SEG;
constexpr int MSM_MERGE_T = 8;
constexpr int MSM_MAX_HEAVY = 1 << 20;
constexpr int MSM_MAX_JOBS = 512;
constexpr int MAX_LANES = 4, CALL_SLOTS = 4;

struct MsmJob {
    const uint32_t* scalars;
    const uint32_t* vmap;
    uint32_t count;
    uint32_t tbl_off;
    uint32_t tbl_count;
    int32_t pt_shift;
    uint32_t c, nw, vw;
    uint32_t ent_off, win_off;
    uint32_t bucket0, bin0, hbits, lbits, tile0, cnt0;
};
struct FinalizeArgs {
    const G1XYZZ* r1; const G2XYZZ* r2;
    const G1XYZZ *foldA, *foldB1, *foldC; const G2XYZZ* foldB2; int fold_n;
    uint8_t dc[MSM_MAX_JOBS / 4], ds[MSM_MAX_JOBS / 4];
    const G1Affine *tblDelta1, *tblAlpha1, *tblBeta1; const G2Affine* tblDelta2;
    G1Affine alpha1; G2Affine beta2;
    const uint8_t* rs; uint8_t* out;
    void* scratch;
    int per; const G1XYZZ* fb4; const G2XYZZ* fb4g2;
    uint8_t* out_xyzz;
};
constexpr int FB4_WIN = 64, FB4_ROW = 15;
struct BlindArgs { const uint32_t* w[2]; const uint32_t* mapA[2]; const uint32_t* mapB[2]; uint32_t nA[2], nB[2]; uint32_t* out[2]; const uint8_t* rs; uint32_t nv; };
constexpr int MSM_TILE = 256, MSM_TILE_SCALARS = 1024;
constexpr uint32_t MSM_MAX_HBITS = 10;
struct MsmJobList {
    MsmJob job[MSM_MAX_JOBS]; int njobs; uint32_t total_buckets, total_entries, total_windows, total_bins, total_tiles, total_tilecnt;
    uint32_t hs, hb, nbig;
    uint32_t hbits_big, hbits_small;
    uint32_t vw_big = 1024;
    uint32_t vw_small = 256;
    void add(const uint32_t* scalars, const uint32_t* vmap, uint32_t count, uint32_t tbl_off, uint32_t tbl_count, int32_t pt_shift, int c) {
        MsmJob& j = job[njobs++];
        uint32_t vw = c >= 16 ? vw_big : vw_small;
        if (vw > (uint32_t)msm_half(c)) vw = (uint32_t)msm_half(c);
        while ((uint32_t)msm_half(c) / vw > max_vw_per_job) vw <<= 1;
        j = MsmJob{scalars, vmap, count, tbl_off, tbl_count, pt_shift, (uint32_t)c, (uint32_t)msm_nw(c), vw, total_entries, total_windows, 0, 0, 0, 0, 0, 0};
        total_entries += count * (uint32_t)msm_nw(c); total_windows += (uint32_t)msm_half(c) / vw;
    }
    uint32_t max_vw_per_job = 256;
    void clear(uint32_t vw_small_jobs = 256, uint32_t vw_big_jobs = 1024, uint32_t max_per_job = 256) { vw_small = vw_small_jobs; vw_big = vw_big_jobs; max_vw_per_job = max_per_job; njobs = 0; total_buckets = total_entries = total_windows = total_bins = total_tiles = total_tilecnt = 0; hs = hb = nbig = 0; }
    bool finish() {
        hs = 0xffffffffu; hb = 0;
        for (int j = 0; j < njobs; j++) { const uint32_t h = 1u << (job[j].c - 1); hs = h < hs ? h : hs; hb = h > hb ? h : hb; }
        nbig = 0; total_buckets = total_bins = total_tiles = total_tilecnt = 0; hbits_big = hbits_small = 0;
        for (int j = 0; j < njobs; j++) {
            MsmJob& q = job[j]; const uint32_t h = 1u << (q.c - 1);
            if (h != hs && h != hb) return false;
            if (h == hb) { if ((uint32_t)j != nbig) return false; nbig++; }
            uint32_t hbits = q.c - 1 < 8 ? q.c - 1 : 8, lbits = q.c - 1 - hbits;
            const uint64_t rows = (uint64_t)q.nw * q.tbl_count;
            while (lbits > 8 || (lbits > 0 && rows >= (1ull << (31 - lbits)))) { lbits--; hbits++; }
            if (hbits > MSM_MAX_HBITS || rows >= (1ull << (31 - lbits))) return false;
            q.hbits = hbits; q.lbits = lbits;
            { uint32_t& cls = h == hb ? hbits_big : hbits_small; cls = (cls == 0 || cls == hbits) ? hbits : 0xffu; }
            q.bucket0 = total_buckets; total_buckets += h;
            q.bin0 = total_bins; total_bins += 1u << hbits;
            const uint32_t nt = (q.count + MSM_TILE_SCALARS - 1) / MSM_TILE_SCALARS;
            q.tile0 = total_tiles; total_tiles += nt; q.cnt0 = total_tilecnt; total_tilecnt += nt << hbits;
        }
        return true;
    }
    ZKC_HD uint32_t id_of(uint32_t d, uint32_t j) const { return job[j].bucket0 + d; }
    ZKC_HD uint32_t job_of_bin(uint32_t bin) const {
        if (hbits_big != 0xffu && hbits_small != 0xffu) {
            const uint32_t lim = nbig << hbits_big;
            return bin < lim ? bin >> hbits_big : nbig + ((bin - lim) >> hbits_small);
        }
        uint32_t lo = 0, hi = (uint32_t)njobs - 1;
        while (lo < hi) { const uint32_t mid = (lo + hi + 1) >> 1; if (job[mid].bin0 <= bin) lo = mid; else hi = mid - 1; }
        return lo;
    }
    ZKC_HD void decode(uint32_t id, uint32_t& d, uint32_t& j) const {
        const uint32_t lim = hb * nbig;
        if (id < lim) { j = id / hb; d = id - j * hb; }
        else { const uint32_t t = id - lim, q = t / hs; j = nbig + q; d = t - q * hs; }
    }
};
struct MsmWindow { uint32_t bucket0, out, per; };

struct MsmWork {
    uint32_t *vals = nullptr, *vals2 = nullptr;
    uint32_t *hist = nullptr, *bin_start = nullptr;
    uint32_t *tilecnt = nullptr; size_t max_tilecnt = 0;
    uint32_t *off = nullptr, *bcnt = nullptr;
    uint32_t *segcnt = nullptr, *segoff = nullptr, *seg2bucket = nullptr, *heavy = nullptr;
    uint32_t *seglen = nullptr, *perm = nullptr;
    uint32_t *scan_blk = nullptr, *lencnt = nullptr; size_t max_lencnt = 0;
    void *partial = nullptr;
    void *wres = nullptr;
    void *results = nullptr;
    void *h_results = nullptr;
    MsmJobList* d_jobs = nullptr;
    MsmWindow* d_windows = nullptr; size_t max_buckets = 0, max_bins = 0, max_windows = 0;
    uint16_t* d_tilejob = nullptr; uint16_t* h_tilejob[2] = {nullptr, nullptr}; size_t max_tiles = 0;
    MsmJobList* h_jobs[2] = {nullptr, nullptr}; MsmWindow* h_windows[2] = {nullptr, nullptr}; hipEvent_t h_ev[2] = {nullptr, nullptr}; int h_next = 0;
    size_t max_entries = 0, max_segments = 0; int max_jobs = 0; size_t xyzz_size = 0;
};
}

struct zkc_lane {
    hipStream_t st = nullptr, st2 = nullptr, fin = nullptr;
    hipStream_t red = nullptr; hipEvent_t ev_red = nullptr;
    zkc::Fr *d_abc = nullptr, *d_t = nullptr; uint32_t* d_p = nullptr;
    void* d_fin = nullptr;
    uint32_t* d_bs = nullptr;
    zkc::MsmWork w1, w2;
    size_t cap_abc = 0, cap_p = 0, cap_fin = 0, cap_bs = 0, bytes = 0; bool made = false;
    hipEvent_t ev_msm = nullptr, ev_msm2 = nullptr, ev_sorted = nullptr, ev_ntt = nullptr, ev_mv = nullptr, ev_acc = nullptr, ev_fin[2] = {nullptr, nullptr}; int npass = 0;
};

struct zkc_zkey {
    zkc_ctx* ctx = nullptr;
    uint32_t nVars = 0, nPub = 0, n = 0, logn = 0, nCoeffs = 0;
    int nLevels = -1;
    zkc::G1Affine alpha1, beta1, delta1;
    zkc::G2Affine beta2, gamma2, delta2;
    std::vector<zkc::G1Affine> ic;
    uint32_t *d_perm = nullptr, *d_rowlen = nullptr, *d_jdptr = nullptr, *d_col = nullptr; zkc::Fr* d_val = nullptr; uint32_t nlong = 0;
    uint32_t n_unit_coeffs = 0;
    zkc::Fr *d_tw_fwd = nullptr, *d_tw_inv = nullptr, *d_coset = nullptr;
    zkc::Fr *d_coset_br = nullptr;
    uint32_t *d_tw_fwd29 = nullptr, *d_tw_inv29 = nullptr;
    zkc::G1Affine* d_g1 = nullptr; zkc::G2Affine* d_g2 = nullptr;
    uint32_t* d_g2_29 = nullptr;
    uint32_t* d_g2_29_lone = nullptr;
    uint32_t offA = 0, offB1 = 0, offC = 0, offH = 0;
    int c_deep = 0; uint32_t offA_deep = 0, offB1_deep = 0, offC_deep = 0; uint32_t* d_g2_29_deep = nullptr;
    int c_h = zkc::MSM_C_BIG;
    int c_sec = zkc::MSM_C_SMALL;
    int max_inflight = 0;
    uint8_t sha256[32] = {0};
    size_t bytes_tables = 0;
    uint8_t fingerprint[32] = {0};
    int nlanes = 1; bool serial_streams = false;
    zkc::G1Affine *d_tblDelta1 = nullptr, *d_tblAlpha1 = nullptr, *d_tblBeta1 = nullptr; zkc::G2Affine* d_tblDelta2 = nullptr;
    uint32_t *d_depths = nullptr, *h_depths = nullptr; size_t depths_cap = 0;
    zkc::G1XYZZ* d_fb4 = nullptr; zkc::G2XYZZ* d_fb4g2 = nullptr; int fb4_bases = 0;
    struct CallSlot {
        uint8_t *d_rs = nullptr, *d_proofs = nullptr; size_t cap = 0;
        uint8_t* h_out = nullptr;
        uint8_t* h_rs = nullptr;
        uint8_t *d_xyzz = nullptr, *h_xyzz = nullptr; std::vector<uint8_t> as_xyzz;
        hipEvent_t ev_done[zkc::MAX_LANES] = {};
        std::vector<hipEvent_t> ev_chunk;
        uint32_t lanes_used = 0;
        int B = 0; bool pending = false;
        uint32_t *d_flags = nullptr, *h_flags = nullptr; size_t flags_cap = 0;
        int32_t* d_status3 = nullptr; size_t status3_cap = 0;
        int early_n = 0; std::vector<uint8_t> early_depth; uint32_t* h_early = nullptr; size_t early_cap = 0;
        const void* arg_wtns = nullptr; uint32_t arg_nw = 0; bool arg_publics = false, arg_inputs = false; int arg_lane0 = -1; hipEvent_t arg_wait = nullptr; std::vector<uint8_t> h_rs_copy;
    } call[zkc::CALL_SLOTS];
    struct Fold {
        std::vector<zkc::G1XYZZ> baseA, baseB1, baseC; std::vector<zkc::G2XYZZ> baseB2;
        std::vector<zkc::G1XYZZ> sufA[2], sufB1[2], sufC[2]; std::vector<zkc::G2XYZZ> sufB2[2];
        struct VMap { uint32_t* d = nullptr; uint32_t offA = 0, nA = 0, offB = 0, nB = 0, offC = 0, nC = 0; };
        std::map<std::pair<int, int>, VMap> vmaps;
        std::vector<uint8_t> infA, infB, infC;
        zkc::G1XYZZ *d_foldA = nullptr, *d_foldB1 = nullptr, *d_foldC = nullptr; zkc::G2XYZZ* d_foldB2 = nullptr;
        bool ready = false;
    } fold;
};

namespace zkc {
int ntt_run(zkc_ctx* ctx, hipStream_t st, const Fr* src, Fr* dst, const uint32_t* tw29, const Fr* scale, int logn, int nvec);
int ntt_make_tw29(zkc_ctx* ctx, const Fr* d_tw, uint32_t count, uint32_t** out);
int ntt_pair_run(zkc_ctx* ctx, hipStream_t st, Fr* data, const uint32_t* tw_inv29, const uint32_t* tw_fwd29, const Fr* scale_br, int logn, int nvec);
int ntt_bitrev_table(zkc_ctx* ctx, const Fr* d_src, Fr** out, int logn);
int msm_work_alloc(zkc_ctx* ctx, MsmWork& w, size_t max_entries, size_t max_buckets, int max_jobs, bool g2);
void msm_work_free(MsmWork& w);
int msm_pass_g1(zkc_zkey* zk, MsmWork& w, const MsmJobList& jl, int slot, bool to_host, hipStream_t st, hipEvent_t ev_sorted = nullptr, hipEvent_t ev_acc = nullptr,
                hipStream_t st_red = nullptr, hipEvent_t ev_red = nullptr);
int msm_pass_g2(zkc_zkey* zk, MsmWork& w, const MsmJobList& jl, int slot, bool to_host, hipStream_t st, hipEvent_t wait_before_acc = nullptr);
int msm_bucket_entries(zkc_ctx* ctx, MsmWork& w, const MsmJobList& jl, hipStream_t st, unsigned long long* d_entry_counter = nullptr);
int msm_build_segments(zkc_ctx* ctx, MsmWork& w, const MsmJobList& jl, uint32_t seg, size_t seg_bound, hipStream_t st);
int finalize_launch(zkc_ctx* ctx, hipStream_t st, const FinalizeArgs& a, int nproofs);
int finalize_tree_g2_launch(zkc_ctx* ctx, hipStream_t st, const FinalizeArgs& a, int nproofs);
int fb4_build(zkc_ctx* ctx, hipStream_t st, const G1XYZZ* d_bases, int nbases, G1XYZZ* d_out, const G2XYZZ& delta2, const G2XYZZ& beta2, const G2XYZZ& beta2_base, G2XYZZ* d_out2);
int blind_scalars_launch(zkc_ctx* ctx, hipStream_t st, const BlindArgs& a, int nproofs);
int prove_batch_begin(zkc_zkey* zk, int cs, const void* d_wtns, uint32_t nWitness, int B, const uint8_t* rs, bool want_publics, const void* d_inputs, int32_t* d_status,
                      int lane0 = -1, hipEvent_t wait_first = nullptr, const uint8_t* host_depths = nullptr, bool no_early = false);
int prove_batch_finish(zkc_zkey* zk, int cs, uint8_t* proofs, uint8_t* publics);
int prove_reserve(zkc_zkey* zk, int inflight);
int zkey_load_opts(zkc_ctx* ctx, const void* zkey_bytes, size_t len, int nlanes, int max_inflight, zkc_zkey** out);
size_t zkey_device_bytes(const zkc_zkey* zk, size_t* tables, size_t* work);
size_t finalize_scratch_bytes(int nproofs);
int msm_precompute_g1(zkc_ctx* ctx, uint32_t count, G1Affine* d_table, int c);
int msm_precompute_g2(zkc_ctx* ctx, uint32_t count, G2Affine* d_table, int c);
int msm_g2_table29(zkc_ctx* ctx, const G2Affine* d_table, uint32_t* d_out, size_t count);
int fold_group_sums_g1(zkc_ctx* ctx, const G1Affine* tbl, const uint32_t* d_scalars, const uint32_t* d_wires, uint32_t nw, int32_t pt_shift,
                       const uint32_t* d_gstart, uint32_t ngroups, G1XYZZ* h_out);
int fold_group_sums_g1_ws(zkc_ctx* ctx, const G1Affine* tbl, const uint32_t* d_scalars, const uint32_t* d_wires, uint32_t nw, const uint32_t* d_gstart, uint32_t ngroups,
                          G1XYZZ* d_tmp , G1XYZZ* d_out , G1XYZZ* h_out);
int fold_group_sums_g2(zkc_ctx* ctx, const G2Affine* tbl, const uint32_t* d_scalars, const uint32_t* d_wires, uint32_t nw, int32_t pt_shift,
                       const uint32_t* d_gstart, uint32_t ngroups, G2XYZZ* h_out);
}
```

Before: 2835.

## Use Shoup precomputed-quotient twiddle multiplication in NTT head and mid stages

Adds a Shoup-style modular multiply for constant twiddles. Each twiddle now stores a precomputed quotient, so a multiply needs only the high partial products against the quotient plus the low products and one correction, with no full Montgomery reduction. New twiddle tables (20 words each) are built at load time for the inverse head and forward mid stages. Butterflies whose whole wavefront has twiddle index zero now skip the multiply. The cost is larger twiddle loads and more register pressure.

```diff
diff --git a/zk-franchise-proof-circuit_amd/csrc/zkc_f29.h b/zk-franchise-proof-circuit_amd/csrc/zkc_f29.h
--- a/zk-franchise-proof-circuit_amd/csrc/zkc_f29.h
+++ b/zk-franchise-proof-circuit_amd/csrc/zkc_f29.h
@@ -184,6 +184,63 @@
     f29_reduce_cols<P>(r, c);
 }
 
+template <class P> struct F29Shoup {
+    static constexpr L9 pbar = [] { L9 r{}; uint64_t br = 0; for (int k = 0; k < 9; k++) { const int64_t v = (k == 8 ? (int64_t)1 << 29 : 0) - (int64_t)P29<P>::limb(k) - (int64_t)br;
+        br = v < 0; r.l[k] = (uint32_t)(v + (br ? (int64_t)1 << 29 : 0)); } return r; }();
+};
+template <class P>
+ZKC_HD void f29_mul_const(uint32_t r[9], const uint32_t v[9], const uint32_t w[9], const uint32_t wq[9]) {
+    constexpr L9 Pb = F29Shoup<P>::pbar;
+    uint64_t h[10], c[9];
+#pragma unroll
+    for (int k = 0; k < 10; k++) h[k] = 0;
+#pragma unroll
+    for (int k = 0; k < 9; k++) c[k] = 0;
+#pragma unroll
+    for (int i = 0; i < 9; i++)
+#pragma unroll
+        for (int j = 0; j < 9; j++) {
+            if (i + j >= 7) h[i + j - 7] += (uint64_t)v[i] * wq[j];
+            if (i + j <= 8) c[i + j] += (uint64_t)v[i] * w[j];
+        }
+    uint32_t q[9];
+    uint64_t carry = (h[0] >> 29) + h[1];
+    carry >>= 29;
+#pragma unroll
+    for (int k = 0; k < 8; k++) { carry += h[k + 2]; q[k] = (uint32_t)carry & F29_MASK; carry >>= 29; }
+    q[8] = (uint32_t)carry;
+#pragma unroll
+    for (int i = 0; i < 9; i++)
+#pragma unroll
+        for (int j = 0; i + j <= 8; j++) c[i + j] += (uint64_t)q[i] * Pb.l[j];
+    carry = 0;
+#pragma unroll
+    for (int k = 0; k < 8; k++) { carry += c[k]; r[k] = (uint32_t)carry & F29_MASK; carry >>= 29; }
+    r[8] = (uint32_t)(carry + c[8]) & F29_MASK;
+}
+template <class P>
+ZKC_HD void f29_shoup_const(uint32_t wq[9], const uint32_t w[9]) {
+    constexpr L9 Pl = F29K<P>::p;
+    uint32_t rem[9];
+#pragma unroll
+    for (int k = 0; k < 9; k++) { rem[k] = w[k]; wq[k] = 0; }
+    for (int bit = 260; bit >= 0; bit--) {
+        uint32_t cin = 0, qin = 0;
+        for (int k = 0; k < 9; k++) {
+            const uint32_t t = (rem[k] << 1) | cin, u = (wq[k] << 1) | qin;
+            cin = k < 8 ? t >> 29 : 0; qin = k < 8 ? u >> 29 : 0;
+            rem[k] = k < 8 ? t & F29_MASK : t; wq[k] = k < 8 ? u & F29_MASK : u;
+        }
+        bool ge = true;
+        for (int k = 8; k >= 0; k--) if (rem[k] != Pl.l[k]) { ge = rem[k] > Pl.l[k]; break; }
+        if (ge) {
+            int64_t br = 0;
+            for (int k = 0; k < 9; k++) { const int64_t t = (int64_t)rem[k] - Pl.l[k] - br; br = t < 0; rem[k] = (uint32_t)(t + (br ? (int64_t)1 << 29 : 0)); }
+            wq[0] |= 1;
+        }
+    }
+}
+
 template <class P>
 ZKC_HD bool f29_is_zero_mod_p(const uint32_t a[9]) {
     const uint32_t k = (a[0] * F29K<P>::pinv) & F29_MASK;
diff --git a/zk-franchise-proof-circuit_amd/csrc/zkc_ntt.hip b/zk-franchise-proof-circuit_amd/csrc/zkc_ntt.hip
--- a/zk-franchise-proof-circuit_amd/csrc/zkc_ntt.hip
+++ b/zk-franchise-proof-circuit_amd/csrc/zkc_ntt.hip
@@ -84,7 +84,7 @@
 }
 
 constexpr int NTT_TILE = 1024;
-constexpr int TW29_WORDS = 12;
+constexpr int TW29_WORDS = 12, TWC_WORDS = 20;
 extern "C" __global__ void __launch_bounds__(256) zkc_tw29(const Fr* __restrict__ tw, uint32_t* __restrict__ out, uint32_t count) {
     const uint32_t i = blockIdx.x * blockDim.x + threadIdx.x;
     if (i >= count) return;
@@ -93,21 +93,49 @@
     uint4* o = reinterpret_cast<uint4*>(out + (size_t)TW29_WORDS * i);
     o[0] = make_uint4(r[0], r[1], r[2], r[3]); o[1] = make_uint4(r[4], r[5], r[6], r[7]); o[2] = make_uint4(r[8], 0, 0, 0);
 }
+extern "C" __global__ void __launch_bounds__(256) zkc_twc29(const Fr* __restrict__ tw, uint32_t* __restrict__ out, uint32_t count) {
+    const uint32_t i = blockIdx.x * blockDim.x + threadIdx.x;
+    if (i >= count) return;
+    uint32_t s[8]; fp_to_std<FrParams>(s, ld_fr(tw + i));
+    const uint32_t w[9] = {slice29<0>(s), slice29<29>(s), slice29<58>(s), slice29<87>(s), slice29<116>(s), slice29<145>(s), slice29<174>(s), slice29<203>(s), slice29<232>(s)};
+    uint32_t wq[9]; f29_shoup_const<FrParams>(wq, w);
+    uint4* o = reinterpret_cast<uint4*>(out + (size_t)TWC_WORDS * i);
+    o[0] = make_uint4(w[0], w[1], w[2], w[3]); o[1] = make_uint4(w[4], w[5], w[6], w[7]); o[2] = make_uint4(w[8], wq[0], wq[1], wq[2]);
+    o[3] = make_uint4(wq[3], wq[4], wq[5], wq[6]); o[4] = make_uint4(wq[7], wq[8], 0, 0);
+}
 struct NttDom { static constexpr L9 D24 = f29_dominator<FrParams>(1u << 29, 1u << 24); static constexpr L9 D27 = f29_dominator<FrParams>(1u << 29, 1u << 27); };
-__device__ __forceinline__ void ntt_ld_w(uint32_t w[9], const uint32_t* __restrict__ tw29, size_t e) {
-    const uint4* wp = reinterpret_cast<const uint4*>(tw29 + (size_t)TW29_WORDS * e);
-    const uint4 w0 = wp[0], w1 = wp[1], w2 = wp[2];
-    w[0] = w0.x; w[1] = w0.y; w[2] = w0.z; w[3] = w0.w; w[4] = w1.x; w[5] = w1.y; w[6] = w1.z; w[7] = w1.w; w[8] = w2.x;
-}
-__device__ __forceinline__ void ntt_bfly(uint32_t* pu, uint32_t* pv, const uint32_t w[9], bool plain, bool carry) {
+template <bool SHOUP> struct NttTw {
+    uint32_t w[SHOUP ? 18 : 9];
+    __device__ __forceinline__ void load(const uint32_t* __restrict__ tw, size_t e) {
+        const uint4* wp = reinterpret_cast<const uint4*>(tw + (size_t)(SHOUP ? TWC_WORDS : TW29_WORDS) * e);
+        const uint4 w0 = wp[0], w1 = wp[1], w2 = wp[2];
+        w[0] = w0.x; w[1] = w0.y; w[2] = w0.z; w[3] = w0.w; w[4] = w1.x; w[5] = w1.y; w[6] = w1.z; w[7] = w1.w; w[8] = w2.x;
+        if constexpr (SHOUP) {
+            const uint4 w3 = wp[3], w4 = wp[4];
+            w[9] = w2.y; w[10] = w2.z; w[11] = w2.w; w[12] = w3.x; w[13] = w3.y; w[14] = w3.z; w[15] = w3.w; w[16] = w4.x; w[17] = w4.y;
+        }
+    }
+    __device__ __forceinline__ void mul(uint32_t t[9], const uint32_t v[9], bool unit) const {
+        if (unit) {
+#pragma unroll
+            for (int i = 0; i < 9; i++) t[i] = v[i];
+            f29_carry(t); f29_reduce_small<FrParams>(t);
+        } else if constexpr (SHOUP) f29_mul_const<FrParams>(t, v, w, w + 9);
+        else f29_mul<FrParams>(t, v, w);
+    }
+};
+template <bool SHOUP>
+__device__ __forceinline__ void ntt_bfly(uint32_t* pu, uint32_t* pv, const uint32_t* __restrict__ tw, size_t e, bool plain, bool carry) {
     uint32_t u[9], v[9], tt[9];
+    NttTw<SHOUP> w;
+    if (!plain) w.load(tw, e);
 #pragma unroll
     for (int i = 0; i < 9; i++) { u[i] = pu[i]; v[i] = pv[i]; }
     if (plain) {
 #pragma unroll
         for (int i = 0; i < 9; i++) { const uint32_t vi = v[i]; v[i] = u[i] + NttDom::D27.l[i] - vi; u[i] += vi; }
     } else {
-        f29_mul<FrParams>(tt, v, w);
+        w.mul(tt, v, __all(e == 0));
 #pragma unroll
         for (int i = 0; i < 9; i++) { v[i] = u[i] + NttDom::D24.l[i] - tt[i]; u[i] += tt[i]; }
     }
@@ -115,24 +143,28 @@
 #pragma unroll
     for (int i = 0; i < 9; i++) { pu[i] = u[i]; pv[i] = v[i]; }
 }
-__device__ __forceinline__ void ntt_r4(uint32_t* p0, uint32_t* p1, uint32_t* p2, uint32_t* p3, const uint32_t wa[9], const uint32_t wb[9], const uint32_t wc[9], bool swap_mid) {
+template <bool SHOUP>
+__device__ __forceinline__ void ntt_r4(uint32_t* p0, uint32_t* p1, uint32_t* p2, uint32_t* p3, const uint32_t* __restrict__ tw, size_t ea, size_t eb, size_t ec) {
     uint32_t a[9], b[9], c[9], d[9], t[9];
+    NttTw<SHOUP> wa, wb, wc;
+    wa.load(tw, ea); wb.load(tw, eb);
+    const bool ua = __all(ea == 0), ub = __all(eb == 0);
 #pragma unroll
     for (int i = 0; i < 9; i++) { a[i] = p0[i]; b[i] = p1[i]; c[i] = p2[i]; d[i] = p3[i]; }
-    f29_mul<FrParams>(t, b, wa);
+    wa.mul(t, b, ua);
 #pragma unroll
     for (int i = 0; i < 9; i++) { b[i] = a[i] + NttDom::D24.l[i] - t[i]; a[i] += t[i]; }
-    f29_mul<FrParams>(t, d, wa);
+    wa.mul(t, d, ua);
 #pragma unroll
     for (int i = 0; i < 9; i++) { d[i] = c[i] + NttDom::D24.l[i] - t[i]; c[i] += t[i]; }
-    f29_mul<FrParams>(t, c, wb);
+    wc.load(tw, ec);
+    wb.mul(t, c, ub);
 #pragma unroll
     for (int i = 0; i < 9; i++) { c[i] = a[i] + NttDom::D24.l[i] - t[i]; a[i] += t[i]; }
-    f29_mul<FrParams>(t, d, wc);
+    wc.mul(t, d, false);
 #pragma unroll
     for (int i = 0; i < 9; i++) { d[i] = b[i] + NttDom::D24.l[i] - t[i]; b[i] += t[i]; }
     f29_carry(a); f29_carry(b); f29_carry(c); f29_carry(d);
-    (void)swap_mid;
 #pragma unroll
     for (int i = 0; i < 9; i++) { p0[i] = a[i]; p1[i] = b[i]; p2[i] = c[i]; p3[i] = d[i]; }
 }
@@ -168,8 +200,7 @@
             const int j = pr & (half - 1), blk = pr >> (t1 - 1);
             const int m0 = (blk << t1) + j, m1 = m0 + half;
             const unsigned k = ((unsigned)j << s0) + lo0 + l;
-            uint32_t w[9]; ntt_ld_w(w, tw29, (size_t)k << (logn - s));
-            ntt_bfly(tile + 9 * (m0 * lo_t + l), tile + 9 * (m1 * lo_t + l), w, s == 1, carry);
+            ntt_bfly<false>(tile + 9 * (m0 * lo_t + l), tile + 9 * (m1 * lo_t + l), tw29, (size_t)k << (logn - s), s == 1, carry);
         }
         __syncthreads();
     };
@@ -181,10 +212,8 @@
             const int j = u & (half - 1), blk = u >> (t - 1);
             const int m = (blk << (t + 1)) + j;
             const unsigned k = ((unsigned)j << s0) + lo0 + l, kh = k + ((unsigned)half << s0);
-            uint32_t wa[9], wb[9], wc[9];
-            ntt_ld_w(wa, tw29, (size_t)k << (logn - s)); ntt_ld_w(wb, tw29, (size_t)k << (logn - s - 1)); ntt_ld_w(wc, tw29, (size_t)kh << (logn - s - 1));
             uint32_t* p = tile + 9 * (m * lo_t + l);
-            ntt_r4(p, p + 9 * half * lo_t, p + 9 * 2 * half * lo_t, p + 9 * 3 * half * lo_t, wa, wb, wc, false);
+            ntt_r4<false>(p, p + 9 * half * lo_t, p + 9 * 2 * half * lo_t, p + 9 * 3 * half * lo_t, tw29, (size_t)k << (logn - s), (size_t)k << (logn - s - 1), (size_t)kh << (logn - s - 1));
         }
         __syncthreads();
     }
@@ -203,7 +232,7 @@
     }
 }
 
-template <int RADIX, class Slot>
+template <int RADIX, bool SHOUP, class Slot>
 __device__ __forceinline__ void ntt_nr_stages(uint32_t* tile, Slot slot, int b, int lo_t, int q0, uint32_t prefix_of_l0, int prefix_per_l, const uint32_t* __restrict__ tw29, int logn, bool fresh) {
     const int mid_n = 1 << b;
     auto tw_of = [&](int q, uint32_t i) -> size_t { return q ? (size_t)((__brev(i) >> (32 - q)) << (logn - q - 1)) : (size_t)0; };
@@ -212,8 +241,7 @@
         const int span = mid_n >> 1, pairs = span * lo_t;
         for (int x = threadIdx.x; x < pairs; x += blockDim.x) {
             const int l = x % lo_t, j = x / lo_t;
-            uint32_t w[9] = {0, 0, 0, 0, 0, 0, 0, 0, 0};
-            ntt_bfly(tile + 9 * slot(j, l), tile + 9 * slot(j + span, l), w, true, true);
+            ntt_bfly<SHOUP>(tile + 9 * slot(j, l), tile + 9 * slot(j + span, l), tw29, 0, true, true);
         }
         __syncthreads();
         r = 1;
@@ -225,9 +253,8 @@
             const int blk = u / hspan, j = u - blk * hspan;
             const int m = blk * 2 * span + j;
             const uint32_t i = ((prefix_of_l0 + (uint32_t)(prefix_per_l * l)) << r) | (uint32_t)blk;
-            uint32_t wa[9], wb[9], wc[9];
-            ntt_ld_w(wa, tw29, tw_of(q, i)); ntt_ld_w(wb, tw29, tw_of(q + 1, 2 * i)); ntt_ld_w(wc, tw29, tw_of(q + 1, 2 * i + 1));
-            ntt_r4(tile + 9 * slot(m, l), tile + 9 * slot(m + span, l), tile + 9 * slot(m + hspan, l), tile + 9 * slot(m + span + hspan, l), wa, wb, wc, false);
+
+            ntt_r4<SHOUP>(tile + 9 * slot(m, l), tile + 9 * slot(m + span, l), tile + 9 * slot(m + hspan, l), tile + 9 * slot(m + span + hspan, l), tw29, tw_of(q, i), tw_of(q + 1, 2 * i), tw_of(q + 1, 2 * i + 1));
         }
         __syncthreads();
     }
@@ -238,8 +265,7 @@
             const int blk = pr / span, j = pr - blk * span;
             const int m0 = blk * 2 * span + j;
             const uint32_t i = ((prefix_of_l0 + (uint32_t)(prefix_per_l * l)) << r) | (uint32_t)blk;
-            uint32_t w[9]; ntt_ld_w(w, tw29, tw_of(q, i));
-            ntt_bfly(tile + 9 * slot(m0, l), tile + 9 * slot(m0 + span, l), w, false, RADIX >= 4 || (r & 1) == 1 || r == b - 1);
+            ntt_bfly<SHOUP>(tile + 9 * slot(m0, l), tile + 9 * slot(m0 + span, l), tw29, tw_of(q, i), false, RADIX >= 4 || (r & 1) == 1 || r == b - 1);
         }
         __syncthreads();
     }
@@ -261,7 +287,7 @@
         for (int k = 0; k < 9; k++) tile[9 * e + k] = t[k];
     }
     __syncthreads();
-    ntt_nr_stages<RADIX>(tile, [lo_t](int mid, int l) { return mid * lo_t + l; }, b, lo_t, q0, prefix, 0, tw29, logn, q0 == 0);
+    ntt_nr_stages<RADIX, true>(tile, [lo_t](int mid, int l) { return mid * lo_t + l; }, b, lo_t, q0, prefix, 0, tw29, logn, q0 == 0);
     for (int e = threadIdx.x; e < elems; e += blockDim.x) {
         const int mid = e / lo_t, l = e - mid * lo_t;
         uint32_t r[9];
@@ -276,7 +302,7 @@
 extern "C" __global__ void __launch_bounds__(256)
 zkc_ntt_nr_head_r4(const Fr* src_all, Fr* dst_all, const uint32_t* __restrict__ tw29, int logn, int q0, int b) { ntt_nr_head_body<4>(src_all, dst_all, tw29, logn, q0, b); }
 extern "C" __global__ void __launch_bounds__(256)
-zkc_ntt_mid(Fr* __restrict__ data_all, const uint32_t* __restrict__ tw_inv29, const uint32_t* __restrict__ tw_fwd29, const Fr* __restrict__ scale_br, int logn) {
+zkc_ntt_mid(Fr* __restrict__ data_all, const uint32_t* __restrict__ tw_inv29, const uint32_t* __restrict__ tw_fwdc, const Fr* __restrict__ scale_br, int logn) {
     Fr* __restrict__ data = data_all + ((size_t)blockIdx.y << logn);
     extern __shared__ uint32_t tile[];
     constexpr int B = 9, MID = 1 << B, NSUB = NTT_TILE / MID;
@@ -288,7 +314,7 @@
         for (int k = 0; k < 9; k++) tile[9 * e + k] = t[k];
     }
     __syncthreads();
-    ntt_nr_stages<4>(tile, [](int mid, int l) { return l * MID + mid; }, B, NSUB, logn - B, (uint32_t)blockIdx.x * NSUB, 1, tw_inv29, logn, false);
+    ntt_nr_stages<4, false>(tile, [](int mid, int l) { return l * MID + mid; }, B, NSUB, logn - B, (uint32_t)blockIdx.x * NSUB, 1, tw_inv29, logn, false);
     for (int e = threadIdx.x; e < NTT_TILE; e += blockDim.x) {
         uint32_t r[9], s29[9], o[9];
 #pragma unroll
@@ -301,8 +327,7 @@
     __syncthreads();
     for (int x = threadIdx.x; x < NTT_TILE / 2; x += blockDim.x) {
         const int l = x / (MID / 2), pr = x - l * (MID / 2);
-        uint32_t w[9] = {0, 0, 0, 0, 0, 0, 0, 0, 0};
-        ntt_bfly(tile + 9 * (l * MID + 2 * pr), tile + 9 * (l * MID + 2 * pr + 1), w, true, true);
+        ntt_bfly<true>(tile + 9 * (l * MID + 2 * pr), tile + 9 * (l * MID + 2 * pr + 1), tw_fwdc, 0, true, true);
     }
     __syncthreads();
     for (int t = 2; t + 1 <= B; t += 2) {
@@ -311,10 +336,8 @@
             const int l = x / (MID / 4), u = x - l * (MID / 4);
             const int j = u & (half - 1), blk = u >> (t - 1);
             const int m = (blk << (t + 1)) + j;
-            uint32_t wa[9], wb[9], wc[9];
-            ntt_ld_w(wa, tw_fwd29, (size_t)j << (logn - t)); ntt_ld_w(wb, tw_fwd29, (size_t)j << (logn - t - 1)); ntt_ld_w(wc, tw_fwd29, (size_t)(j + half) << (logn - t - 1));
             uint32_t* p = tile + 9 * (l * MID + m);
-            ntt_r4(p, p + 9 * half, p + 9 * 2 * half, p + 9 * 3 * half, wa, wb, wc, false);
+            ntt_r4<true>(p, p + 9 * half, p + 9 * 2 * half, p + 9 * 3 * half, tw_fwdc, (size_t)j << (logn - t), (size_t)j << (logn - t - 1), (size_t)(j + half) << (logn - t - 1));
         }
         __syncthreads();
     }
@@ -338,16 +361,16 @@
     ZKC_HIP_CHECK(ctx, hipGetLastError());
     return ZKC_OK;
 }
-int ntt_pair_run(zkc_ctx* ctx, hipStream_t st, Fr* data, const uint32_t* tw_inv29, const uint32_t* tw_fwd29, const Fr* scale_br, int logn, int nvec) {
+int ntt_pair_run(zkc_ctx* ctx, hipStream_t st, Fr* data, const uint32_t* tw_inv29, const uint32_t* tw_fwd29, const uint32_t* tw_invc, const uint32_t* tw_fwdc, const Fr* scale_br, int logn, int nvec) {
     if (logn < 12 || logn > 27) return zkc_fail(ctx, ZKC_ERR_BAD_ARG, "ntt_pair_run: 12 <= logn <= 27");
     const int bh = logn - 9;
     const int b1 = bh <= 9 ? bh : (bh + 1) / 2, b2 = bh - b1;
     const unsigned blocks = (1u << logn) / NTT_TILE;
     static const int radix = [] { const char* e = getenv("ZKC_NTT_RADIX"); return e ? atoi(e) : 4; }();
     auto head = radix >= 4 ? zkc_ntt_nr_head_r4 : zkc_ntt_nr_head;
-    hipLaunchKernelGGL(head, dim3(blocks, nvec), dim3(256), (size_t)NTT_TILE * 36, st, (const Fr*)data, data, tw_inv29, logn, 0, b1);
-    if (b2) hipLaunchKernelGGL(head, dim3(blocks, nvec), dim3(256), (size_t)NTT_TILE * 36, st, (const Fr*)data, data, tw_inv29, logn, b1, b2);
-    hipLaunchKernelGGL(zkc_ntt_mid, dim3(blocks, nvec), dim3(256), (size_t)NTT_TILE * 36, st, data, tw_inv29, tw_fwd29, scale_br, logn);
+    hipLaunchKernelGGL(head, dim3(blocks, nvec), dim3(256), (size_t)NTT_TILE * 36, st, (const Fr*)data, data, tw_invc, logn, 0, b1);
+    if (b2) hipLaunchKernelGGL(head, dim3(blocks, nvec), dim3(256), (size_t)NTT_TILE * 36, st, (const Fr*)data, data, tw_invc, logn, b1, b2);
+    hipLaunchKernelGGL(zkc_ntt_mid, dim3(blocks, nvec), dim3(256), (size_t)NTT_TILE * 36, st, data, tw_inv29, tw_fwdc, scale_br, logn);
     hipLaunchKernelGGL(zkc_ntt_pass, dim3(blocks, nvec), dim3(256), (size_t)NTT_TILE * 36, st, (const Fr*)data, data, tw_fwd29, (const Fr*)nullptr, logn, 9, b1, 0);
     if (b2) hipLaunchKernelGGL(zkc_ntt_pass, dim3(blocks, nvec), dim3(256), (size_t)NTT_TILE * 36, st, (const Fr*)data, data, tw_fwd29, (const Fr*)nullptr, logn, 9 + b1, b2, 0);
     hipError_t e = hipGetLastError();
@@ -355,9 +378,9 @@
     return ZKC_OK;
 }
 
-int ntt_make_tw29(zkc_ctx* ctx, const Fr* d_tw, uint32_t count, uint32_t** out) {
-    ZKC_HIP_CHECK(ctx, hipMalloc((void**)out, (size_t)count * TW29_WORDS * 4));
-    hipLaunchKernelGGL(zkc_tw29, dim3((count + 255) / 256), dim3(256), 0, ctx->stream, d_tw, *out, count);
+int ntt_make_tw29(zkc_ctx* ctx, const Fr* d_tw, uint32_t count, uint32_t** out, bool shoup) {
+    ZKC_HIP_CHECK(ctx, hipMalloc((void**)out, (size_t)count * (shoup ? TWC_WORDS : TW29_WORDS) * 4));
+    hipLaunchKernelGGL(shoup ? zkc_twc29 : zkc_tw29, dim3((count + 255) / 256), dim3(256), 0, ctx->stream, d_tw, *out, count);
     ZKC_HIP_CHECK(ctx, hipGetLastError());
     ZKC_HIP_CHECK(ctx, hipStreamSynchronize(ctx->stream));
     return ZKC_OK;
diff --git a/zk-franchise-proof-circuit_amd/csrc/zkc_prove.hip b/zk-franchise-proof-circuit_amd/csrc/zkc_prove.hip
--- a/zk-franchise-proof-circuit_amd/csrc/zkc_prove.hip
+++ b/zk-franchise-proof-circuit_amd/csrc/zkc_prove.hip
@@ -83,7 +83,7 @@
     ZKC_LOCK(zk->ctx);
     (void)hipSetDevice(zk->ctx->device);
     (void)hipStreamSynchronize(zk->ctx->stream);
-    void* ptrs[] = {zk->d_perm, zk->d_rowlen, zk->d_jdptr, zk->d_col, zk->d_val, zk->d_tw_fwd, zk->d_tw_inv, zk->d_tw_fwd29, zk->d_tw_inv29, zk->d_coset, zk->d_coset_br, zk->d_g1, zk->d_g2, zk->d_g2_29, zk->d_g2_29_lone, zk->d_g2_29_deep,
+    void* ptrs[] = {zk->d_perm, zk->d_rowlen, zk->d_jdptr, zk->d_col, zk->d_val, zk->d_tw_fwd, zk->d_tw_inv, zk->d_tw_fwd29, zk->d_tw_inv29, zk->d_tw_fwdc, zk->d_tw_invc, zk->d_coset, zk->d_coset_br, zk->d_g1, zk->d_g2, zk->d_g2_29, zk->d_g2_29_lone, zk->d_g2_29_deep,
                     zk->d_tblDelta1, zk->d_tblAlpha1, zk->d_tblBeta1, zk->d_tblDelta2, zk->d_fb4, zk->d_fb4g2, zk->d_depths};
     for (void* p : ptrs) if (p) (void)hipFree(p);
     for (auto& kv : zk->fold.vmaps) if (kv.second.d) (void)hipFree(kv.second.d);
@@ -258,6 +258,7 @@
         ZKC_UP(zk->d_tw_inv, b.data(), b.size() * sizeof(Fr));
         ZKC_UP(zk->d_coset, cs.data(), cs.size() * sizeof(Fr));
         if ((rc = ntt_make_tw29(ctx, zk->d_tw_fwd, n / 2, &zk->d_tw_fwd29)) || (rc = ntt_make_tw29(ctx, zk->d_tw_inv, n / 2, &zk->d_tw_inv29))) return bail(rc);
+        if ((rc = ntt_make_tw29(ctx, zk->d_tw_fwd, n / 2, &zk->d_tw_fwdc, true)) || (rc = ntt_make_tw29(ctx, zk->d_tw_inv, n / 2, &zk->d_tw_invc, true))) return bail(rc);
         if ((rc = ntt_bitrev_table(ctx, zk->d_coset, &zk->d_coset_br, (int)zk->logn))) return bail(rc);
     }
     auto c_for = [](size_t W) { return msm_c_for(W); };
@@ -484,7 +485,7 @@
     int rc;
     static const bool ntt_two_transforms = getenv("ZKC_NTT_SEPARATE") != nullptr;
     if (!ntt_two_transforms && zk->logn >= 12 && zk->logn <= 27) {
-        if ((rc = ntt_pair_run(ctx, st, L.d_abc, zk->d_tw_inv29, zk->d_tw_fwd29, zk->d_coset_br, (int)zk->logn, 3 * nb))) return rc;
+        if ((rc = ntt_pair_run(ctx, st, L.d_abc, zk->d_tw_inv29, zk->d_tw_fwd29, zk->d_tw_invc, zk->d_tw_fwdc, zk->d_coset_br, (int)zk->logn, 3 * nb))) return rc;
     } else {
         if ((rc = ntt_run(ctx, st, L.d_abc, L.d_t, zk->d_tw_inv29, zk->d_coset, (int)zk->logn, 3 * nb))) return rc;
         if ((rc = ntt_run(ctx, st, L.d_t, L.d_abc, zk->d_tw_fwd29, nullptr, (int)zk->logn, 3 * nb))) return rc;
diff --git a/zk-franchise-proof-circuit_amd/csrc/zkc_prover.h b/zk-franchise-proof-circuit_amd/csrc/zkc_prover.h
--- a/zk-franchise-proof-circuit_amd/csrc/zkc_prover.h
+++ b/zk-franchise-proof-circuit_amd/csrc/zkc_prover.h
@@ -144,6 +144,7 @@
     zkc::Fr *d_tw_fwd = nullptr, *d_tw_inv = nullptr, *d_coset = nullptr;
     zkc::Fr *d_coset_br = nullptr;
     uint32_t *d_tw_fwd29 = nullptr, *d_tw_inv29 = nullptr;
+    uint32_t *d_tw_fwdc = nullptr, *d_tw_invc = nullptr;
     zkc::G1Affine* d_g1 = nullptr; zkc::G2Affine* d_g2 = nullptr;
     uint32_t* d_g2_29 = nullptr;
     uint32_t* d_g2_29_lone = nullptr;
@@ -186,8 +187,8 @@
 
 namespace zkc {
 int ntt_run(zkc_ctx* ctx, hipStream_t st, const Fr* src, Fr* dst, const uint32_t* tw29, const Fr* scale, int logn, int nvec);
-int ntt_make_tw29(zkc_ctx* ctx, const Fr* d_tw, uint32_t count, uint32_t** out);
-int ntt_pair_run(zkc_ctx* ctx, hipStream_t st, Fr* data, const uint32_t* tw_inv29, const uint32_t* tw_fwd29, const Fr* scale_br, int logn, int nvec);
+int ntt_make_tw29(zkc_ctx* ctx, const Fr* d_tw, uint32_t count, uint32_t** out, bool shoup = false);
+int ntt_pair_run(zkc_ctx* ctx, hipStream_t st, Fr* data, const uint32_t* tw_inv29, const uint32_t* tw_fwd29, const uint32_t* tw_invc, const uint32_t* tw_fwdc, const Fr* scale_br, int logn, int nvec);
 int ntt_bitrev_table(zkc_ctx* ctx, const Fr* d_src, Fr** out, int logn);
 int msm_work_alloc(zkc_ctx* ctx, MsmWork& w, size_t max_entries, size_t max_buckets, int max_jobs, bool g2);
 void msm_work_free(MsmWork& w);
```

Result: no change. 2843 (median of 6 runs) (+0.3%).
